# zoongahn/jodalroB-twoTower

Hardware: AMD Instinct MI355X
Metric: training pairs/sec at batch 8192 (embedding-lookup HBM GB/s in roofline) (higher is better)
Workload: dtype bf16 MFMA operands, f32 accumulate; f32 tables, master weights and activations (the tower input x, which the GEMMs round to bf16 anyway, is stored bf16)

## Files before the change

include/twotower.h:

```cpp
#ifndef TWOTOWER_H_
#define TWOTOWER_H_

#include <stddef.h>
#include <stdint.h>

#ifdef __cplusplus
extern "C" {
#endif

#define TT_ABI_VERSION 2

#define TT_OK 0
#define TT_ERR_INVALID_ARG (-1)
#define TT_ERR_HIP (-2)
#define TT_ERR_WORKSPACE (-3)
#define TT_ERR_UNSUPPORTED (-4)
#define TT_ERR_DEVICE (-5)

#define TT_F32 0
#define TT_BF16 1

#define TT_MAX_SIDES 4
#define TT_MAX_HIDDEN 8

// ... 15 lines not shown
#define TT_OPT_CHAINED 6
#define TT_OPT_LOOKUP_NT 7
#define TT_OPT_CHAIN_SPIN 8
#define TT_OPT_RETRIEVE_SPLITS 9
#define TT_OPT_FUSE_SCORE_TAIL 10
int tt_ctx_set_option(tt_ctx* ctx, int32_t option, int32_t value);
#define TT_DEVERR_CHAIN_TIMEOUT 1u
#define TT_DEVERR_ROW_RANGE 2u
int tt_ctx_check_device_errors(tt_ctx* ctx, tt_stream stream);
int tt_handover_retarget(tt_ctx* ctx, void* graph_exec, void* node);
int tt_handover_captured_node(tt_ctx* ctx, void** node);
int tt_flush_deferred(tt_ctx* ctx, tt_stream stream);
int tt_flush_deferred_slabs(tt_ctx* ctx, tt_stream stream);
int tt_deferred_pending(const tt_ctx* ctx);

typedef struct tt_embed_side {
  const int64_t* ids;
  const int64_t* key_row_offset;
  const int64_t* key_vocab;
  void* out;
  int64_t ld_out;
  int32_t K;
  int32_t out_dtype;
} tt_embed_side;

int tt_embed_lookup_set_profile(tt_ctx* ctx, uint64_t* ring_dev, int32_t n_slots);
int tt_embed_lookup_fwd(tt_ctx* ctx, const float* table, int64_t table_rows, int32_t E,
                        const tt_embed_side* sides, int32_t n_sides, int64_t B, int32_t* rows_out,
                        tt_stream stream);
int tt_embed_lookup_rows_fwd(tt_ctx* ctx, const float* table, int64_t table_rows, int32_t E,
                             const tt_embed_side* sides, int32_t n_sides, int64_t B, const int32_t* rows,
                             tt_stream stream);

size_t tt_dedup_workspace_bytes(int64_t M);
int tt_dedup_plan(tt_ctx* ctx, const int32_t* rows, int64_t M, int64_t table_rows,
                  int32_t* sorted_src, int32_t* unique_rows, int32_t* seg_offsets, int32_t* n_unique,
                  void* workspace, size_t workspace_bytes, tt_stream stream);

size_t tt_dedup_keyed_workspace_bytes(int64_t M, int32_t n_keys);
int tt_dedup_plan_keyed(tt_ctx* ctx, const int32_t* rows, const int32_t* side_K ,
                        int32_t n_sides, int64_t B, int32_t* sorted_src, int32_t* unique_rows,
                        int32_t* seg_offsets, int32_t* n_unique, void* workspace, size_t workspace_bytes,
                        tt_stream stream);

int tt_dedup_plan_keyed_km(tt_ctx* ctx, const int32_t* rows_km, const int32_t* side_K ,
                           int32_t n_sides, int64_t B, int32_t* sorted_src, int32_t* unique_rows,
                           int32_t* seg_offsets, int32_t* n_unique, void* workspace, size_t workspace_bytes,
                           tt_stream stream);

int tt_dedup_plan_keyed_long(tt_ctx* ctx, const int32_t* rows, int32_t rows_key_major, const int32_t* side_K ,
                             int32_t n_sides, int64_t B, int32_t E, int32_t* sorted_src, int32_t* unique_rows,
                             int32_t* seg_offsets, int32_t* n_unique, void* grad_workspace, size_t grad_workspace_bytes,
                             void* workspace, size_t workspace_bytes, tt_stream stream);

#define TT_GRAD_SPARSE 0
#define TT_GRAD_DENSE_SET 1
#define TT_GRAD_DENSE_ACC 2
#define TT_GRAD_SHORT_SEGMENTS 0x100
#define TT_GRAD_PLANNED 0x200
#define TT_GRAD_DEFER_FINISH 0x400

typedef struct tt_grad_src {
  const void* d_out;
  int64_t ld;
  int32_t K;
  int32_t dtype;
} tt_grad_src;

size_t tt_embed_grad_workspace_bytes(int64_t M, int32_t E);
int tt_embed_grad_bwd(tt_ctx* ctx, const tt_grad_src* srcs, int32_t n_srcs, int64_t B, int32_t E,
                      const int32_t* sorted_src, const int32_t* seg_offsets,
                      const int32_t* unique_rows, const int32_t* n_unique, int64_t M, int32_t mode,
                      float* out, int32_t* counters, void* workspace, size_t workspace_bytes, tt_stream stream);

void tt_adam_hparams(int64_t step, float lr, float beta1, float beta2, float eps, float weight_decay,
                     float out6[6]);
int tt_adam_dense_step(tt_ctx* ctx, float* p, const float* g, float* m, float* v, int64_t n,
                       int64_t step, float lr, float beta1, float beta2, float eps,
                       float weight_decay, const float* hparams_dev, tt_stream stream);
typedef struct tt_adam_tensor {
  float* p;
  const float* g;
  float* m;
  float* v;
  int64_t n;
} tt_adam_tensor;
int tt_adam_multi_step(tt_ctx* ctx, const tt_adam_tensor* tensors , int32_t n_tensors,
                       int64_t step, float lr, float beta1, float beta2, float eps,
                       float weight_decay, const float* hparams_dev, tt_stream stream);
int tt_sparse_adam_step(tt_ctx* ctx, float* table, float* m, float* v, int64_t table_rows, int32_t E,
                        const int32_t* unique_rows, const float* grad_rows, const int32_t* n_unique,
                        int64_t M, int64_t step, float lr, float beta1, float beta2, float eps,
                        float weight_decay, const float* hparams_dev, tt_stream stream);

int tt_adam_fused_step(tt_ctx* ctx, const tt_adam_tensor* tensors, int32_t n_tensors, float* table, float* m, float* v,
                       int64_t table_rows, int32_t E, const int32_t* unique_rows, const float* grad_rows, const int32_t* n_unique, int64_t M,
                       int64_t step, float lr, float beta1, float beta2, float eps, float weight_decay,
                       const float* hparams_dev, tt_stream stream);

int tt_adam_fused_step_finish(tt_ctx* ctx, const tt_adam_tensor* tensors, int32_t n_tensors, float* table, float* m, float* v,
                              int64_t table_rows, int32_t E, const int32_t* unique_rows, float* grad_rows, const int32_t* n_unique,
                              int64_t M, const int32_t* seg_offsets, void* grad_workspace, size_t grad_workspace_bytes,
                              int64_t step, float lr, float beta1, float beta2, float eps, float weight_decay,
                              const float* hparams_dev, tt_stream stream);

int tt_rowwise_adagrad_sparse_step(tt_ctx* ctx, float* table, float* sum, int64_t table_rows, int32_t E,
                                   const int32_t* unique_rows, const float* grad_rows, const int32_t* n_unique, int64_t M,
                                   float lr, float eps, float weight_decay, const float* hparams_dev, tt_stream stream);
int tt_rowwise_adagrad_dense_step(tt_ctx* ctx, float* table, float* sum, const float* grad, int64_t table_rows, int32_t E,
                                  float lr, float eps, float weight_decay, const float* hparams_dev, tt_stream stream);
int tt_adam_rowwise_adagrad_fused_step(tt_ctx* ctx, const tt_adam_tensor* tensors, int32_t n_tensors, int64_t step, float lr,
                                       float beta1, float beta2, float eps, float weight_decay, const float* hparams_dev,
                                       float* table, float* sum, int64_t table_rows, int32_t E, const int32_t* unique_rows,
                                       const float* grad_rows, const int32_t* n_unique, int64_t M, float table_lr,
                                       float table_eps, float table_weight_decay, const float* table_hparams_dev,
                                       tt_stream stream);
int tt_adam_rowwise_adagrad_fused_step_finish(tt_ctx* ctx, const tt_adam_tensor* tensors, int32_t n_tensors, int64_t step,
                                              float lr, float beta1, float beta2, float eps, float weight_decay,
                                              const float* hparams_dev, float* table, float* sum, int64_t table_rows, int32_t E,
                                              const int32_t* unique_rows, float* grad_rows, const int32_t* n_unique, int64_t M,
                                              const int32_t* seg_offsets, void* grad_workspace, size_t grad_workspace_bytes,
                                              float table_lr, float table_eps, float table_weight_decay,
                                              const float* table_hparams_dev, tt_stream stream);
int tt_embed_grad_finish(tt_ctx* ctx, int32_t E, const int32_t* seg_offsets, int64_t M, float* out, void* workspace,
                         size_t workspace_bytes, tt_stream stream);

typedef struct tt_tower_params {
  int32_t din, h0, kcat_e, n_hidden, d_out;
  int32_t hidden[TT_MAX_HIDDEN];
  const float* w_proj;
  const float* b_proj;
  const float* w[TT_MAX_HIDDEN];
  const float* b[TT_MAX_HIDDEN];
  const float* bn_w[TT_MAX_HIDDEN];
  const float* bn_b[TT_MAX_HIDDEN];
  float* bn_rm[TT_MAX_HIDDEN];
  float* bn_rv[TT_MAX_HIDDEN];
  int64_t* bn_nbt[TT_MAX_HIDDEN];
  const float* w_out;
  const float* b_out;
  int32_t compute_dtype;
  int32_t x_dtype;
  int32_t dx_dtype;
  int32_t flags;
  int32_t sync_phase;
  int32_t sync_ranks;
  int64_t rng_row_offset;
  const void* w_proj_bf16;
  const void* w_bf16[TT_MAX_HIDDEN];
} tt_tower_params;
#define TT_TOWER_UNFUSED_TAIL 1
#define TT_TOWER_UNFUSED_FRONT 2
#define TT_TOWER_UNFUSED_BACK 4

typedef struct tt_tower_acts {
  const float* dense;
  void* x;
  float* pre[TT_MAX_HIDDEN];
  float* act[TT_MAX_HIDDEN];
  float* mean[TT_MAX_HIDDEN];
  float* rstd[TT_MAX_HIDDEN];
  float* y;
  float* emb;
  void* emb_packed;
  float emb_pack_scale;
  float* bn_sync_local;
  const float* bn_sync_all;
  int64_t bn_sync_stride;
} tt_tower_acts;

typedef struct tt_tower_grads {
  float* w_proj;
  float* b_proj;
  float* w[TT_MAX_HIDDEN];
  float* b[TT_MAX_HIDDEN];
  float* bn_w[TT_MAX_HIDDEN];
  float* bn_b[TT_MAX_HIDDEN];
  float* w_out;
  float* b_out;
  void* d_x;
  float* scratch[TT_MAX_HIDDEN];
  float* d_y;
  float* s_sync_local;
  const float* s_sync_all;
  int64_t s_sync_stride;
} tt_tower_grads;

size_t tt_tower_workspace_bytes(const tt_tower_params* p, int64_t B);
int tt_tower_mlp_fwd(tt_ctx* ctx, const tt_tower_params* p, const tt_tower_acts* a, int64_t B,
                     int32_t train, float dropout_p, uint64_t seed, const uint64_t* seed_dev,
                     void* workspace, size_t workspace_bytes, tt_stream stream);
int tt_tower_mlp_bwd(tt_ctx* ctx, const tt_tower_params* p, const tt_tower_acts* a,
                     const float* d_emb, const tt_tower_grads* g, int64_t B, int32_t train,
                     float dropout_p, uint64_t seed, const uint64_t* seed_dev, void* workspace,
                     size_t workspace_bytes, tt_stream stream);

int tt_towers_mlp_fwd(tt_ctx* ctx, int32_t n, const tt_tower_params* const* p, const tt_tower_acts* const* a,
                      int64_t B, int32_t train, float dropout_p, uint64_t seed, const uint64_t* seed_dev,
                      void* const* workspaces, const size_t* workspace_bytes, tt_stream stream);
int tt_towers_mlp_bwd(tt_ctx* ctx, int32_t n, const tt_tower_params* const* p, const tt_tower_acts* const* a,
                      const float* const* d_emb, const tt_tower_grads* const* g, int64_t B, int32_t train,
                      float dropout_p, uint64_t seed, const uint64_t* seed_dev, void* const* workspaces,
                      const size_t* workspace_bytes, tt_stream stream);

int tt_score_dir_fwd(tt_ctx* ctx, const float* A, const float* Bm, int64_t Ra, int64_t Rb, int32_t D,
                     float inv_t, float shift, int64_t diag_offset, float* sumexp, float* diag,
                     int32_t* rank, float* sumscore ,
                     tt_stream stream);
int tt_score_loss_finish(tt_ctx* ctx, int64_t B, float shift, const float* rowsum,
                         const float* colsum, const float* diag, const int32_t* row_rank,
                         const int32_t* col_rank, const float* sumscore, float* out8,
                         float* loss_out , tt_stream stream);
int tt_score_dir_bwd(tt_ctx* ctx, const float* A, const float* Bm, int64_t Ra, int64_t Rb, int32_t D,
                     float inv_t, float shift, int64_t diag_offset, const float* sumexp_a,
                     const float* sumexp_b, const float* d_loss, float scale, float* dA,
                     tt_stream stream);
typedef struct tt_score_fwd_dir {
  const void* A_packed;
  const void* B_packed;
  int64_t Ra, Rb, diag_offset;
  float* sumexp;
  float* diag;
  int32_t* rank;
  float* sumscore;
  int32_t rank_mode;
  float ab_scale;
  float* inv_sumexp;
} tt_score_fwd_dir;
typedef struct tt_score_bwd_dir {
  const void* A_packed;
  const void* B_packed;
  int64_t Ra, Rb, diag_offset;
  const float* sumexp_a;
  const float* sumexp_b;
  float* dA;
  float ab_scale;
  float b_scale;
  const float* inv_a;
  const float* inv_b;
} tt_score_bwd_dir;
size_t tt_score_pack_bytes(int64_t R, int32_t D);
float tt_score_unit_scale(float inv_t);
int tt_score_pack_bf16(tt_ctx* ctx, const float* X, int64_t R, int32_t D, float scale, void* packed, tt_stream stream);
int tt_score_pack2_bf16(tt_ctx* ctx, const float* X0, int64_t R0, void* packed0, const float* X1, int64_t R1,
                        void* packed1, int32_t D, float scale0, float scale1, tt_stream stream);
int tt_score_fwd_bf16(tt_ctx* ctx, const tt_score_fwd_dir* dirs, int32_t n_dirs, int32_t D, float inv_t,
                      float shift, tt_stream stream);
int tt_score_bwd_bf16(tt_ctx* ctx, const tt_score_bwd_dir* dirs, int32_t n_dirs, int32_t D, float inv_t,
                      float shift, const float* d_loss, float scale, tt_stream stream);
size_t tt_score_fwd_sym_workspace_bytes(int64_t B, int32_t D);
int tt_score_fwd_sym_bf16(tt_ctx* ctx, const void* N_packed, const void* C_packed, int64_t B, int32_t D, float inv_t,
                          float shift, float ab_scale, int32_t want_rank, float* rowsum, float* colsum, float* inv_row,
                          float* inv_col, float* diag, int32_t* row_rank, float* out8, float* loss_out, void* workspace,
                          size_t workspace_bytes, tt_stream stream);
size_t tt_score_pack_fp8_bytes(int64_t R, int32_t D);
int tt_score_pack2_fp8(tt_ctx* ctx, const float* X0, int64_t R0, void* packed0, const float* X1, int64_t R1,
                       void* packed1, int32_t D, float scale0, float scale1, tt_stream stream);
int tt_score_fwd_sym_fp8(tt_ctx* ctx, const void* N_packed, const void* C_packed, int64_t B, int32_t D, float inv_t,
                         float shift, float ab_scale, int32_t want_rank, float* rowsum, float* colsum, float* inv_row,
                         float* inv_col, float* diag, int32_t* row_rank, float* out8, float* loss_out, void* workspace,
                         size_t workspace_bytes, tt_stream stream);
int tt_score_bwd_fp8(tt_ctx* ctx, const tt_score_bwd_dir* dirs, int32_t n_dirs, int32_t D, float inv_t,
                     float shift, const float* d_loss, float scale, tt_stream stream);
size_t tt_score_pack_x3_bytes(int64_t R, int32_t D);
int tt_score_pack2_bf16x3(tt_ctx* ctx, const float* X0, int64_t R0, void* packed0, const float* X1, int64_t R1,
                          void* packed1, int32_t D, float scale0, float scale1, tt_stream stream);
int tt_score_fwd_sym_bf16x3(tt_ctx* ctx, const void* N_packed, const void* C_packed, int64_t B, int32_t D, float inv_t,
                            float shift, float ab_scale, int32_t want_rank, float* rowsum, float* colsum, float* inv_row,
                            float* inv_col, float* diag, int32_t* row_rank, float* out8, float* loss_out, void* workspace,
                            size_t workspace_bytes, tt_stream stream);
int tt_score_fwd_bf16x3(tt_ctx* ctx, const tt_score_fwd_dir* dirs, int32_t n_dirs, int32_t D, float inv_t,
                        float shift, tt_stream stream);
int tt_score_bwd_bf16x3(tt_ctx* ctx, const tt_score_bwd_dir* dirs, int32_t n_dirs, int32_t D, float inv_t,
                        float shift, const float* d_loss, float scale, tt_stream stream);
typedef struct tt_score_bwd_lq {
  const float* w_a;
  const float* w_b;
} tt_score_bwd_lq;
int tt_score_fwd_sym_bf16_lq(tt_ctx* ctx, const void* N_packed, const void* C_packed, int64_t B, int32_t D, float inv_t,
                             float shift, float ab_scale, int32_t want_rank, const float* lq_n, const float* lq_c, float* rowsum,
                             float* colsum, float* inv_row, float* inv_col, float* w_n, float* w_c, float* diag,
                             int32_t* row_rank, float* out8, float* loss_out, void* workspace, size_t workspace_bytes,
                             tt_stream stream);
int tt_score_fwd_sym_bf16x3_lq(tt_ctx* ctx, const void* N_packed, const void* C_packed, int64_t B, int32_t D, float inv_t,
                               float shift, float ab_scale, int32_t want_rank, const float* lq_n, const float* lq_c,
                               float* rowsum, float* colsum, float* inv_row, float* inv_col, float* w_n, float* w_c,
                               float* diag, int32_t* row_rank, float* out8, float* loss_out, void* workspace,
                               size_t workspace_bytes, tt_stream stream);
int tt_score_bwd_bf16_lq(tt_ctx* ctx, const tt_score_bwd_dir* dirs, const tt_score_bwd_lq* lq, int32_t n_dirs, int32_t D,
                         float inv_t, float shift, const float* d_loss, float scale, tt_stream stream);
int tt_score_bwd_bf16x3_lq(tt_ctx* ctx, const tt_score_bwd_dir* dirs, const tt_score_bwd_lq* lq, int32_t n_dirs, int32_t D,
                           float inv_t, float shift, const float* d_loss, float scale, tt_stream stream);
int tt_score_dir_fwd_lq(tt_ctx* ctx, const float* A, const float* Bm, int64_t Ra, int64_t Rb, int32_t D, float inv_t,
                        float shift, int64_t diag_offset, const float* lq_b, float* sumexp, float* diag, int32_t* rank,
                        float* sumscore, tt_stream stream);
int tt_score_loss_finish_lq(tt_ctx* ctx, int64_t B, float shift, const float* lq_n, const float* lq_c, const float* rowsum,
                            const float* colsum, const float* diag, const int32_t* row_rank, const int32_t* col_rank,
                            const float* sumscore, float* out8, float* loss_out, tt_stream stream);
int tt_score_dir_bwd_lq(tt_ctx* ctx, const float* A, const float* Bm, int64_t Ra, int64_t Rb, int32_t D, float inv_t,
                        float shift, int64_t diag_offset, const float* lq_a, const float* lq_b, const float* sumexp_a,
                        const float* sumexp_b, const float* d_loss, float scale, float* dA, tt_stream stream);
int tt_score_fwd_sym_bf16_mask(tt_ctx* ctx, const void* N_packed, const void* C_packed, int64_t B, int32_t D, float inv_t,
                               float shift, float ab_scale, int32_t want_rank, const int32_t* ent_n, const int32_t* ent_c,
                               const float* lq_n, const float* lq_c, float* rowsum, float* colsum, float* inv_row,
                               float* inv_col, float* w_n, float* w_c, float* diag, int32_t* row_rank, float* out8,
                               float* loss_out, void* workspace, size_t workspace_bytes, tt_stream stream);
int tt_score_bwd_bf16_mask(tt_ctx* ctx, const tt_score_bwd_dir* dirs, const int32_t* ent_n, const int32_t* ent_c,
                           const tt_score_bwd_lq* lq, int32_t n_dirs, int32_t D, float inv_t, float shift,
                           const float* d_loss, float scale, tt_stream stream);
int tt_score_dir_fwd_mask(tt_ctx* ctx, const float* A, const float* Bm, int64_t Ra, int64_t Rb, int32_t D, float inv_t,
                          float shift, int64_t diag_offset, const int32_t* ent_n, const int32_t* ent_c, const float* lq_b,
                          float* sumexp, float* diag, int32_t* rank, float* sumscore, tt_stream stream);
int tt_score_dir_bwd_mask(tt_ctx* ctx, const float* A, const float* Bm, int64_t Ra, int64_t Rb, int32_t D, float inv_t,
                          float shift, int64_t diag_offset, const int32_t* ent_n, const int32_t* ent_c, const float* lq_a,
                          const float* lq_b, const float* sumexp_a, const float* sumexp_b, const float* d_loss, float scale,
                          float* dA, tt_stream stream);
int tt_score_prepare_pw(tt_ctx* ctx, const float* w, int64_t B, float* g_out, tt_stream stream);
int tt_score_fwd_sym_bf16_pw(tt_ctx* ctx, const void* N_packed, const void* C_packed, int64_t B, int32_t D, float inv_t,
                             float shift, float ab_scale, int32_t want_rank, const float* g, const int32_t* ent_n,
                             const int32_t* ent_c, const float* lq_n, const float* lq_c, float* rowsum, float* colsum,
                             float* inv_row, float* inv_col, float* w_n, float* w_c, float* diag, int32_t* row_rank,
                             float* out8, float* loss_out, void* workspace, size_t workspace_bytes, tt_stream stream);
int tt_score_bwd_bf16_pw(tt_ctx* ctx, const tt_score_bwd_dir* dirs, const float* g, const int32_t* ent_n,
                         const int32_t* ent_c, const tt_score_bwd_lq* lq, int32_t n_dirs, int32_t D, float inv_t, float shift,
                         const float* d_loss, float scale, tt_stream stream);
int tt_score_loss_finish_pw(tt_ctx* ctx, int64_t B, float shift, const float* g, const float* lq_n, const float* lq_c,
                            const float* rowsum, const float* colsum, const float* diag, const int32_t* row_rank,
                            const int32_t* col_rank, const float* sumscore, float* out8, float* loss_out, tt_stream stream);
int tt_score_dir_bwd_pw(tt_ctx* ctx, const float* A, const float* Bm, int64_t Ra, int64_t Rb, int32_t D, float inv_t,
                        float shift, int64_t diag_offset, const float* g, const int32_t* ent_n, const int32_t* ent_c,
                        const float* lq_a, const float* lq_b, const float* sumexp_a, const float* sumexp_b,
                        const float* d_loss, float scale, float* dA, tt_stream stream);
size_t tt_score_dense_workspace_bytes(int64_t B, int32_t D);
int tt_score_dense_fwd(tt_ctx* ctx, const float* N, const float* Cm, int64_t B, int32_t D, float inv_t, int32_t loss_type,
                       float label_smoothing, float* S, float* stats, int32_t* hit, float* out8, float* loss_out,
                       tt_stream stream);
int tt_score_dense_bwd(tt_ctx* ctx, const float* N, const float* Cm, int64_t B, int32_t D, float inv_t, int32_t loss_type,
                       float label_smoothing, float* S, const float* stats, const float* d_loss, float* dN, float* dC,
                       void* workspace, size_t workspace_bytes, tt_stream stream);
int tt_score_matrix(tt_ctx* ctx, const float* A, const float* Bm, int64_t Ra, int64_t Rb, int32_t D,
                    float inv_t, float* S, int64_t lds, tt_stream stream);
int tt_diag_rank_rows(tt_ctx* ctx, const float* S, int64_t R, int64_t Ccols, int64_t lds,
                      int64_t diag_offset, int32_t* rank, tt_stream stream);
int tt_topk_rows(tt_ctx* ctx, const float* S, int64_t R, int64_t Ccols, int64_t lds, int32_t k,
                 float* vals, int64_t* idx, tt_stream stream);

size_t tt_retrieve_workspace_bytes(int64_t nQ, int64_t nC, int32_t D, int32_t k);
int tt_retrieve_topk_bf16(tt_ctx* ctx, const void* Q_packed, int64_t nQ, const void* C_packed, int64_t nC, int32_t D, int32_t k,
                          const void* positives, int32_t positives_i64, float* vals, int64_t* idx, int32_t* rank, void* workspace,
                          size_t workspace_bytes, tt_stream stream);
int tt_retrieve_topk_f32(tt_ctx* ctx, const float* Q, int64_t nQ, const float* Cm, int64_t nC, int32_t D, float inv_t, int32_t k,
                         const void* positives, int32_t positives_i64, float* vals, int64_t* idx, int32_t* rank, void* workspace,
// ... 99 lines not shown
```

jodalrob-twotower_amd/_lib.py:

```python
from __future__ import annotations

import ctypes as C
from pathlib import Path
from typing import Optional

import torch

_PKG = Path(__file__).resolve().parent
LIB_PATH = _PKG / "libtwotower_hip.so"

TT_F32, TT_BF16 = 0, 1
TT_MAX_SIDES, TT_MAX_HIDDEN = 4, 8
TT_GRAD_SPARSE, TT_GRAD_DENSE_SET, TT_GRAD_DENSE_ACC = 0, 1, 2
TT_TOWER_UNFUSED_TAIL = 1
TT_TOWER_UNFUSED_FRONT = 2
TT_TOWER_UNFUSED_BACK = 4
TT_GRAD_SHORT_SEGMENTS = 0x100
TT_GRAD_PLANNED = 0x200
TT_GRAD_DEFER_FINISH = 0x400

vp = C.c_void_p
i32, i64, f32, u64, sz = C.c_int32, C.c_int64, C.c_float, C.c_uint64, C.c_size_t


class EmbedSide(C.Structure):
    _fields_ = [("ids", vp), ("key_row_offset", vp), ("key_vocab", vp), ("out", vp), ("ld_out", i64),
                ("K", i32), ("out_dtype", i32)]


class StoreSide(C.Structure):
    _fields_ = [("entity", vp), ("entity_stride", i64), ("dense_store", vp), ("cat_store", vp), ("dense_out", vp), ("ids_out", vp),
                ("dense_dim", i32), ("n_rows", i32)]


TT_MAX_CVT = 8


class CvtList(C.Structure):
    _fields_ = [("n", i32), ("reserved", i32), ("src", vp * TT_MAX_CVT), ("dst", vp * TT_MAX_CVT), ("count", i64 * TT_MAX_CVT)]


class IngestLookup(C.Structure):
    _fields_ = [("table", vp), ("table_rows", i64), ("E", i32), ("reserved", i32)]


class GradSrc(C.Structure):
    _fields_ = [("d_out", vp), ("ld", i64), ("K", i32), ("dtype", i32)]


class AdamTensor(C.Structure):
    _fields_ = [("p", vp), ("g", vp), ("m", vp), ("v", vp), ("n", i64)]


class ScoreFwdDir(C.Structure):
    _fields_ = [("A_packed", vp), ("B_packed", vp), ("Ra", i64), ("Rb", i64), ("diag_offset", i64),
                ("sumexp", vp), ("diag", vp), ("rank", vp), ("sumscore", vp), ("rank_mode", i32), ("ab_scale", f32), ("inv_sumexp", vp)]


class ScoreBwdDir(C.Structure):
    _fields_ = [("A_packed", vp), ("B_packed", vp), ("Ra", i64), ("Rb", i64), ("diag_offset", i64),
                ("sumexp_a", vp), ("sumexp_b", vp), ("dA", vp), ("ab_scale", f32), ("b_scale", f32), ("inv_a", vp), ("inv_b", vp)]


class ScoreBwdLq(C.Structure):
    _fields_ = [("w_a", vp), ("w_b", vp)]


_H = vp * TT_MAX_HIDDEN


class TowerParams(C.Structure):
    _fields_ = [("din", i32), ("h0", i32), ("kcat_e", i32), ("n_hidden", i32), ("d_out", i32),
                ("hidden", i32 * TT_MAX_HIDDEN),
                ("w_proj", vp), ("b_proj", vp), ("w", _H), ("b", _H), ("bn_w", _H), ("bn_b", _H),
                ("bn_rm", _H), ("bn_rv", _H), ("bn_nbt", _H), ("w_out", vp), ("b_out", vp), ("compute_dtype", i32),
                ("x_dtype", i32), ("dx_dtype", i32), ("flags", i32),
                ("sync_phase", i32), ("sync_ranks", i32), ("rng_row_offset", i64),
                ("w_proj_bf16", vp), ("w_bf16", _H)]


class TowerActs(C.Structure):
    _fields_ = [("dense", vp), ("x", vp), ("pre", _H), ("act", _H), ("mean", _H), ("rstd", _H), ("y", vp), ("emb", vp), ("emb_packed", vp), ("emb_pack_scale", f32),
                ("bn_sync_local", vp), ("bn_sync_all", vp), ("bn_sync_stride", i64)]


class TowerGrads(C.Structure):
    _fields_ = [("w_proj", vp), ("b_proj", vp), ("w", _H), ("b", _H), ("bn_w", _H), ("bn_b", _H),
                ("w_out", vp), ("b_out", vp), ("d_x", vp), ("scratch", _H), ("d_y", vp), ("s_sync_local", vp), ("s_sync_all", vp), ("s_sync_stride", i64)]


SIGNATURES = {
    "tt_abi_version": (C.c_int, []),
    "tt_ctx_create": (C.c_int, [C.c_int, C.POINTER(vp)]),
    "tt_ctx_destroy": (C.c_int, [vp]),
    "tt_last_error_string": (C.c_char_p, []),
    "tt_ctx_num_cus": (C.c_int, [vp]),
    "tt_embed_lookup_set_profile": (C.c_int, [vp, vp, i32]),
    "tt_embed_lookup_fwd": (C.c_int, [vp, vp, i64, i32, C.POINTER(EmbedSide), i32, i64, vp, vp]),
    "tt_embed_lookup_rows_fwd": (C.c_int, [vp, vp, i64, i32, C.POINTER(EmbedSide), i32, i64, vp, vp]),
    "tt_dedup_workspace_bytes": (sz, [i64]),
    "tt_dedup_plan": (C.c_int, [vp, vp, i64, i64, vp, vp, vp, vp, vp, sz, vp]),
    "tt_dedup_keyed_workspace_bytes": (sz, [i64, i32]),
    "tt_dedup_plan_keyed": (C.c_int, [vp, vp, C.POINTER(i32), i32, i64, vp, vp, vp, vp, vp, sz, vp]),
    "tt_dedup_plan_keyed_km": (C.c_int, [vp, vp, C.POINTER(i32), i32, i64, vp, vp, vp, vp, vp, sz, vp]),
    "tt_dedup_plan_keyed_long": (C.c_int, [vp, vp, i32, C.POINTER(i32), i32, i64, i32, vp, vp, vp, vp, vp, sz, vp, sz, vp]),
    "tt_embed_grad_workspace_bytes": (sz, [i64, i32]),
    "tt_embed_grad_bwd": (C.c_int, [vp, C.POINTER(GradSrc), i32, i64, i32, vp, vp, vp, vp, i64, i32, vp, vp, vp, sz, vp]),
    "tt_adam_hparams": (None, [i64, f32, f32, f32, f32, f32, C.POINTER(f32 * 6)]),
    "tt_adam_dense_step": (C.c_int, [vp, vp, vp, vp, vp, i64, i64, f32, f32, f32, f32, f32, vp, vp]),
    "tt_adam_multi_step": (C.c_int, [vp, C.POINTER(AdamTensor), i32, i64, f32, f32, f32, f32, f32, vp, vp]),
    "tt_sparse_adam_step": (C.c_int, [vp, vp, vp, vp, i64, i32, vp, vp, vp, i64, i64, f32, f32, f32, f32, f32, vp, vp]),
    "tt_adam_fused_step": (C.c_int, [vp, C.POINTER(AdamTensor), i32, vp, vp, vp, i64, i32, vp, vp, vp, i64, i64, f32, f32, f32, f32,
                                     f32, vp, vp]),
    "tt_adam_fused_step_finish": (C.c_int, [vp, C.POINTER(AdamTensor), i32, vp, vp, vp, i64, i32, vp, vp, vp, i64, vp, vp, sz, i64, f32,
                                            f32, f32, f32, f32, vp, vp]),
    "tt_rowwise_adagrad_sparse_step": (C.c_int, [vp, vp, vp, i64, i32, vp, vp, vp, i64, f32, f32, f32, vp, vp]),
    "tt_rowwise_adagrad_dense_step": (C.c_int, [vp, vp, vp, vp, i64, i32, f32, f32, f32, vp, vp]),
    "tt_adam_rowwise_adagrad_fused_step": (C.c_int, [vp, C.POINTER(AdamTensor), i32, i64, f32, f32, f32, f32, f32, vp, vp, vp, i64, i32,
                                                     vp, vp, vp, i64, f32, f32, f32, vp, vp]),
    "tt_adam_rowwise_adagrad_fused_step_finish": (C.c_int, [vp, C.POINTER(AdamTensor), i32, i64, f32, f32, f32, f32, f32, vp, vp, vp,
                                                            i64, i32, vp, vp, vp, i64, vp, vp, sz, f32, f32, f32, vp, vp]),
    "tt_embed_grad_finish": (C.c_int, [vp, i32, vp, i64, vp, vp, sz, vp]),
    "tt_ctx_set_option": (C.c_int, [vp, i32, i32]),
    "tt_flush_deferred": (C.c_int, [vp, vp]),
    "tt_ctx_check_device_errors": (C.c_int, [vp, vp]),
    "tt_handover_retarget": (C.c_int, [vp, vp, vp]),
    "tt_handover_captured_node": (C.c_int, [vp, C.POINTER(vp)]),
    "tt_deferred_pending": (C.c_int, [vp]),
    "tt_launch_count": (C.c_uint64, []),
    "tt_flush_deferred_slabs": (C.c_int, [vp, vp]),
    "tt_tower_workspace_bytes": (sz, [C.POINTER(TowerParams), i64]),
    "tt_tower_mlp_fwd": (C.c_int, [vp, C.POINTER(TowerParams), C.POINTER(TowerActs), i64, i32, f32, u64, vp, vp, sz, vp]),
    "tt_tower_mlp_bwd": (C.c_int, [vp, C.POINTER(TowerParams), C.POINTER(TowerActs), vp, C.POINTER(TowerGrads), i64, i32,
                                   f32, u64, vp, vp, sz, vp]),
    "tt_towers_mlp_fwd": (C.c_int, [vp, i32, C.POINTER(C.POINTER(TowerParams)), C.POINTER(C.POINTER(TowerActs)), i64, i32, f32, u64,
                                    vp, C.POINTER(vp), C.POINTER(sz), vp]),
    "tt_towers_mlp_bwd": (C.c_int, [vp, i32, C.POINTER(C.POINTER(TowerParams)), C.POINTER(C.POINTER(TowerActs)), C.POINTER(vp),
                                    C.POINTER(C.POINTER(TowerGrads)), i64, i32, f32, u64, vp, C.POINTER(vp), C.POINTER(sz), vp]),
    "tt_score_dir_fwd": (C.c_int, [vp, vp, vp, i64, i64, i32, f32, f32, i64, vp, vp, vp, vp, vp]),
    "tt_score_loss_finish": (C.c_int, [vp, i64, f32, vp, vp, vp, vp, vp, vp, vp, vp, vp]),
    "tt_score_dir_bwd": (C.c_int, [vp, vp, vp, i64, i64, i32, f32, f32, i64, vp, vp, vp, f32, vp, vp]),
    "tt_score_pack_bytes": (sz, [i64, i32]),
    "tt_score_unit_scale": (f32, [f32]),
    "tt_score_pack_bf16": (C.c_int, [vp, vp, i64, i32, f32, vp, vp]),
    "tt_score_pack2_bf16": (C.c_int, [vp, vp, i64, vp, vp, i64, vp, i32, f32, f32, vp]),
    "tt_score_fwd_bf16": (C.c_int, [vp, C.POINTER(ScoreFwdDir), i32, i32, f32, f32, vp]),
    "tt_score_bwd_bf16": (C.c_int, [vp, C.POINTER(ScoreBwdDir), i32, i32, f32, f32, vp, f32, vp]),
    "tt_score_pack_fp8_bytes": (sz, [i64, i32]),
    "tt_score_pack2_fp8": (C.c_int, [vp, vp, i64, vp, vp, i64, vp, i32, f32, f32, vp]),
    "tt_score_fwd_sym_fp8": (C.c_int, [vp, vp, vp, i64, i32, f32, f32, f32, i32, vp, vp, vp, vp, vp, vp, vp, vp, vp, sz, vp]),
    "tt_score_bwd_fp8": (C.c_int, [vp, C.POINTER(ScoreBwdDir), i32, i32, f32, f32, vp, f32, vp]),
    "tt_score_fwd_sym_workspace_bytes": (sz, [i64, i32]),
    "tt_score_fwd_sym_bf16": (C.c_int, [vp, vp, vp, i64, i32, f32, f32, f32, i32, vp, vp, vp, vp, vp, vp, vp, vp, vp, sz, vp]),
    "tt_score_pack_x3_bytes": (sz, [i64, i32]),
    "tt_score_pack2_bf16x3": (C.c_int, [vp, vp, i64, vp, vp, i64, vp, i32, f32, f32, vp]),
    "tt_score_fwd_sym_bf16x3": (C.c_int, [vp, vp, vp, i64, i32, f32, f32, f32, i32, vp, vp, vp, vp, vp, vp, vp, vp, vp, sz, vp]),
    "tt_score_fwd_bf16x3": (C.c_int, [vp, C.POINTER(ScoreFwdDir), i32, i32, f32, f32, vp]),
    "tt_score_bwd_bf16x3": (C.c_int, [vp, C.POINTER(ScoreBwdDir), i32, i32, f32, f32, vp, f32, vp]),
    "tt_score_fwd_sym_bf16_lq": (C.c_int, [vp, vp, vp, i64, i32, f32, f32, f32, i32, vp, vp, vp, vp, vp, vp, vp, vp, vp, vp, vp, vp, vp,
                                           sz, vp]),
    "tt_score_fwd_sym_bf16x3_lq": (C.c_int, [vp, vp, vp, i64, i32, f32, f32, f32, i32, vp, vp, vp, vp, vp, vp, vp, vp, vp, vp, vp, vp, vp,
                                             sz, vp]),
    "tt_score_bwd_bf16_lq": (C.c_int, [vp, C.POINTER(ScoreBwdDir), C.POINTER(ScoreBwdLq), i32, i32, f32, f32, vp, f32, vp]),
    "tt_score_bwd_bf16x3_lq": (C.c_int, [vp, C.POINTER(ScoreBwdDir), C.POINTER(ScoreBwdLq), i32, i32, f32, f32, vp, f32, vp]),
    "tt_score_dir_fwd_lq": (C.c_int, [vp, vp, vp, i64, i64, i32, f32, f32, i64, vp, vp, vp, vp, vp, vp]),
    "tt_score_loss_finish_lq": (C.c_int, [vp, i64, f32, vp, vp, vp, vp, vp, vp, vp, vp, vp, vp, vp]),
    "tt_score_dir_bwd_lq": (C.c_int, [vp, vp, vp, i64, i64, i32, f32, f32, i64, vp, vp, vp, vp, vp, f32, vp, vp]),
    "tt_score_fwd_sym_bf16_mask": (C.c_int, [vp, vp, vp, i64, i32, f32, f32, f32, i32, vp, vp, vp, vp, vp, vp, vp, vp, vp, vp, vp, vp, vp,
                                             vp, vp, sz, vp]),
    "tt_score_bwd_bf16_mask": (C.c_int, [vp, C.POINTER(ScoreBwdDir), vp, vp, C.POINTER(ScoreBwdLq), i32, i32, f32, f32, vp, f32, vp]),
    "tt_score_dir_fwd_mask": (C.c_int, [vp, vp, vp, i64, i64, i32, f32, f32, i64, vp, vp, vp, vp, vp, vp, vp, vp]),
    "tt_score_dir_bwd_mask": (C.c_int, [vp, vp, vp, i64, i64, i32, f32, f32, i64, vp, vp, vp, vp, vp, vp, vp, f32, vp, vp]),
    "tt_score_prepare_pw": (C.c_int, [vp, vp, i64, vp, vp]),
    "tt_score_fwd_sym_bf16_pw": (C.c_int, [vp, vp, vp, i64, i32, f32, f32, f32, i32, vp, vp, vp, vp, vp, vp, vp, vp, vp, vp, vp, vp, vp, vp,
                                           vp, vp, sz, vp]),
    "tt_score_bwd_bf16_pw": (C.c_int, [vp, C.POINTER(ScoreBwdDir), vp, vp, vp, C.POINTER(ScoreBwdLq), i32, i32, f32, f32, vp, f32, vp]),
    "tt_score_loss_finish_pw": (C.c_int, [vp, i64, f32, vp, vp, vp, vp, vp, vp, vp, vp, vp, vp, vp, vp]),
    "tt_score_dir_bwd_pw": (C.c_int, [vp, vp, vp, i64, i64, i32, f32, f32, i64, vp, vp, vp, vp, vp, vp, vp, vp, f32, vp, vp]),
    "tt_score_matrix": (C.c_int, [vp, vp, vp, i64, i64, i32, f32, vp, i64, vp]),
    "tt_score_dense_workspace_bytes": (sz, [i64, i32]),
    "tt_score_dense_fwd": (C.c_int, [vp, vp, vp, i64, i32, f32, i32, f32, vp, vp, vp, vp, vp, vp]),
    "tt_score_dense_bwd": (C.c_int, [vp, vp, vp, i64, i32, f32, i32, f32, vp, vp, vp, vp, vp, vp, sz, vp]),
    "tt_diag_rank_rows": (C.c_int, [vp, vp, i64, i64, i64, i64, vp, vp]),
    "tt_topk_rows": (C.c_int, [vp, vp, i64, i64, i64, i32, vp, vp, vp]),
    "tt_retrieve_workspace_bytes": (sz, [i64, i64, i32, i32]),
    "tt_retrieve_topk_bf16": (C.c_int, [vp, vp, i64, vp, i64, i32, i32, vp, i32, vp, vp, vp, vp, sz, vp]),
    "tt_retrieve_topk_f32": (C.c_int, [vp, vp, i64, vp, i64, i32, f32, i32, vp, i32, vp, vp, vp, vp, sz, vp]),
    "tt_excl_retrieve_topk_bf16": (C.c_int, [vp, vp, i64, vp, i64, i32, i32, vp, i32, vp, vp, vp, vp, vp, vp, sz, vp]),
    "tt_excl_retrieve_topk_f32": (C.c_int, [vp, vp, i64, vp, i64, i32, f32, i32, vp, i32, vp, vp, vp, vp, vp, vp, sz, vp]),
    "tt_filt_retrieve_topk_bf16": (C.c_int, [vp, vp, i64, vp, i64, i32, i32, vp, i32, vp, vp, vp, vp, vp, vp, i32, vp, vp, vp, sz, vp]),
    "tt_filt_retrieve_topk_f32": (C.c_int, [vp, vp, i64, vp, i64, i32, f32, i32, vp, i32, vp, vp, vp, vp, vp, vp, i32, vp, vp, vp, sz,
                                            vp]),
    "tt_linear_fwd": (C.c_int, [vp, vp, i64, vp, vp, vp, i64, i64, i32, i32, i32, vp]),
    "tt_route_workspace_bytes": (sz, [i64, i32]),
    "tt_route_bucket": (C.c_int, [vp, vp, vp, i64, i32, i32, C.POINTER(i32), i32, vp, vp, vp, vp, vp, vp, sz, vp]),
    "tt_route_expand": (C.c_int, [vp, vp, vp, vp, vp, i64, vp, vp]),
    "tt_route_bucket_expand": (C.c_int, [vp, vp, vp, i64, i32, i32, C.POINTER(i32), i32, vp, vp, vp, vp, vp, vp, sz, vp, vp, vp, vp]),
    "tt_dedup_plan_runs": (C.c_int, [vp, vp, i32, i64, i64, vp, vp, vp, vp, vp, sz, vp]),
    "tt_gather_rows": (C.c_int, [vp, vp, i64, i32, vp, i64, vp, i32, vp]),
    "tt_copy_multi": (C.c_int, [vp, i32, C.POINTER(vp), C.POINTER(vp), C.POINTER(i64), vp]),
    "tt_batch_ingest": (C.c_int, [vp, i32, C.POINTER(vp), C.POINTER(vp), C.POINTER(i64), C.POINTER(EmbedSide), i32, i64, vp, vp, i64, C.POINTER(CvtList), vp]),
    "tt_batch_gather": (C.c_int, [vp, vp, i64, vp, i32, vp, i32, vp, vp, vp]),
    "tt_batch_ingest_store": (C.c_int, [vp, i32, C.POINTER(vp), C.POINTER(vp), C.POINTER(i64), C.POINTER(EmbedSide), C.POINTER(StoreSide), i32,
                                        i64, vp, vp, vp, i64, C.POINTER(CvtList), vp]),
    "tt_batch_ingest_lookup": (C.c_int, [vp, i32, C.POINTER(vp), C.POINTER(vp), C.POINTER(i64), C.POINTER(EmbedSide), i32, i64, vp,
                                         C.POINTER(IngestLookup), C.POINTER(CvtList), vp]),
    "tt_batch_ingest_store_lookup": (C.c_int, [vp, i32, C.POINTER(vp), C.POINTER(vp), C.POINTER(i64), C.POINTER(EmbedSide), C.POINTER(StoreSide),
                                               i32, i64, vp, vp, C.POINTER(IngestLookup), C.POINTER(CvtList), vp]),
}

_lib: Optional[C.CDLL] = None
_ctxs: dict = {}
_defer_on: set = set()
_riders_on: dict = {}
_workspaces: dict = {}


class TwoTowerHipError(RuntimeError):
    pass


def load() -> C.CDLL:
    global _lib
    if _lib is None:
        if not LIB_PATH.exists():
            raise TwoTowerHipError(
                f"{LIB_PATH} is missing: build it with `python -c 'import __graft_entry__ as g; g.build()'` "
                "(hipcc --offload-arch=gfx950).  There is no CPU fallback for the two-tower hot path.")
        lib = C.CDLL(str(LIB_PATH))
        for name, (res, args) in SIGNATURES.items():
            fn = getattr(lib, name)
            fn.restype, fn.argtypes = res, args
        _lib = lib
    return _lib


def check(rc: int, what: str = ""):
    if rc != 0:
        msg = load().tt_last_error_string().decode("utf-8", "replace")
        raise TwoTowerHipError(f"{what or 'twotower call'} failed (status {rc}): {msg}")


def ctx(device: torch.device) -> vp:
    device = torch.device(device)
    if device.type != "cuda":
        raise TwoTowerHipError(f"the two-tower hot path runs on MI355X only; got tensors on '{device}' "
                               "(no CPU fallback exists)")
    idx = device.index if device.index is not None else torch.cuda.current_device()
    if idx not in _ctxs:
        h = vp()
        check(load().tt_ctx_create(idx, C.byref(h)), "tt_ctx_create")
        _ctxs[idx] = h
    return _ctxs[idx]


def stream(device: torch.device) -> vp:
    return vp(torch.cuda.current_stream(device).cuda_stream)


def ptr(t: Optional[torch.Tensor]) -> vp:
    return vp(0 if t is None else t.data_ptr())


TT_OPT_DEFER_SLAB_REDUCE = 1
TT_OPT_KEYED_PARTS = 2
TT_OPT_SCORE_BWD_ROWS_MIN = 3
TT_OPT_DEFER_RIDERS = 4
TT_OPT_FP8_GRAD = 5
TT_OPT_CHAINED = 6
TT_OPT_LOOKUP_NT = 7
TT_OPT_CHAIN_SPIN = 8
TT_OPT_RETRIEVE_SPLITS = 9
TT_OPT_FUSE_SCORE_TAIL = 10


def set_option(device: torch.device, option: int, value: int):
    check(load().tt_ctx_set_option(ctx(device), int(option), int(value)), "tt_ctx_set_option")


def set_defer_slab_reduce(device: torch.device, on: bool):
    check(load().tt_ctx_set_option(ctx(device), TT_OPT_DEFER_SLAB_REDUCE, 1 if on else 0), "tt_ctx_set_option")
    idx = torch.device(device).index
    (_defer_on.add if on else _defer_on.discard)(idx if idx is not None else torch.cuda.current_device())
    if not on:
        flush_deferred(device)


def set_defer_riders(device: torch.device, on, loss_only: bool = False):
    mask = (2 if loss_only else 3) if on else 0
# ... 78 lines not shown
```

jodalrob-twotower_amd/config.py:

```python
from __future__ import annotations

import os
from dataclasses import dataclass


@dataclass
class Settings:
    score_dtype: str = "fp32"
    mlp_dtype: str = "fp32"
    embedding_grad: str = "dense"
    sync_debug: bool = False
    tower_io_dtype: str = "x"
    tower_unfused_tail: bool = False
    tower_unfused_front: bool = False
    tower_unfused_back: bool = False
    tower_pack: bool = True
    graph_ingest: bool = True
    graph_weight_shadows: bool = True
    graph_ingest_rows: bool = True
    graph_ingest_lookup: bool = False
    grad_planned: bool = True

    @classmethod
    def from_env(cls) -> "Settings":
        e = os.environ
        return cls(score_dtype=e.get("TT_SCORE_DTYPE", "fp32"), mlp_dtype=e.get("TT_MLP_DTYPE", "fp32"),
                   embedding_grad=e.get("TT_EMBEDDING_GRAD", "dense"), sync_debug=e.get("TT_SYNC_DEBUG", "0") not in ("", "0"))


settings = Settings.from_env()
```

jodalrob-twotower_amd/csrc/tt_tower.hip:

```cpp
#include "tt_deferred.h"
#include "tt_tail_bwd.h"

namespace {

using namespace tttail;

constexpr int kThreads = 256;

struct BnStatArgs {
  const float* pre; int B, H, rows_per_chunk, nchunks; float* partial; float* mean; float* rstd; float* rm; float* rv; int64_t* nbt;
  int64_t pstride = 0;
};

__global__ __launch_bounds__(kThreads) void bn_stats_partial_kernel(Batch<BnStatArgs> batch) {
  const BnStatArgs& a = batch.a[blockIdx.z];
  const int H = a.H;
  if ((int)blockIdx.x * 64 >= H || (int)blockIdx.y >= a.nchunks) return;
  __shared__ Wf sh[4][64];
  const int c = blockIdx.x * 64 + (threadIdx.x & 63), rl = threadIdx.x >> 6;
  const int r0 = blockIdx.y * a.rows_per_chunk, r1 = min(a.B, r0 + a.rows_per_chunk);
  Wf w{0.f, 0.f, 0.f};
  if (c < H && r0 + rl < r1) {
    const float x0 = fmaxf(a.pre[(int64_t)(r0 + rl) * H + c], 0.f);
    float s = 0.f, q = 0.f, cnt = 0.f;
// ... 217 lines not shown
  for (int r = 0; r < RW; ++r)
#pragma unroll
    for (int j = 0; j < NC; ++j) v[r][j] = row0 + r < a.B ? a.y[(int64_t)(row0 + r) * D + lane + 64 * j] : 0.f;
#pragma unroll
  for (int r = 0; r < RW; ++r) {
    float ss = mul_rn(v[r][0], v[r][0]);
#pragma unroll
    for (int j = 1; j < NC; ++j) ss = __builtin_fmaf(v[r][j], v[r][j], ss);
    const float den = fmaxf(sqrtf(wave_sum(ss)), kNormEps);
    if (row0 + r < a.B) {
#pragma unroll
      for (int j = 0; j < NC; ++j) a.out[(int64_t)(row0 + r) * D + lane + 64 * j] = v[r][j] / den;
    }
  }
}

template <int NC, int RW>
__global__ __launch_bounds__(kThreads) void l2norm_bwd_fast_kernel(Batch<NormArgs> batch) {
  const NormArgs& a = batch.a[blockIdx.y];
  const int lane = threadIdx.x & 63, D = 64 * NC;
  const int row0 = (blockIdx.x * 4 + (threadIdx.x >> 6)) * RW;
  if (row0 >= a.B) return;
  float y[RW][NC], e[RW][NC], d[RW][NC];
#pragma unroll
  for (int r = 0; r < RW; ++r)
#pragma unroll
    for (int j = 0; j < NC; ++j) {
      const bool ok = row0 + r < a.B;
      const int64_t i = (int64_t)(row0 + r) * D + lane + 64 * j;
      y[r][j] = ok ? a.y[i] : 0.f;
      e[r][j] = ok ? a.emb_in[i] : 0.f;
      d[r][j] = ok ? a.d_emb[i] : 0.f;
    }
#pragma unroll
  for (int r = 0; r < RW; ++r) {
    float ss = mul_rn(y[r][0], y[r][0]), dot = mul_rn(e[r][0], d[r][0]);
#pragma unroll
    for (int j = 1; j < NC; ++j) {
      ss = __builtin_fmaf(y[r][j], y[r][j], ss);
      dot = __builtin_fmaf(e[r][j], d[r][j], dot);
    }
    const float nrm = sqrtf(wave_sum(ss));
    dot = wave_sum(dot);
    const float den = fmaxf(nrm, kNormEps);
    if (row0 + r < a.B) {
#pragma unroll
      for (int j = 0; j < NC; ++j)
        a.out[(int64_t)(row0 + r) * D + lane + 64 * j] = nrm > kNormEps ? (d[r][j] - e[r][j] * dot) / den : d[r][j] / den;
    }
  }
}

template <bool BWD>
static bool launch_l2norm_fast(hipStream_t st, const Batch<NormArgs>& na, int n, int64_t B) {
  const int D = na.a[0].D;
  for (int t = 1; t < n; ++t)
    if (na.a[t].D != D || na.a[t].B != na.a[0].B) return false;
  if (D % 64 != 0 || D < 64 || D > 256) return false;
  constexpr int RW = BWD ? 2 : 4;
  const dim3 grid((unsigned)tt_cdiv(B, 4 * RW), (unsigned)n);
  auto launch = [&](auto kernel) { kernel<<<grid, kThreads, 0, st>>>(na); };
#define TT_L2(NC)                                        \
  do {                                                   \
    if (BWD) launch(l2norm_bwd_fast_kernel<NC, RW>);     \
    else launch(l2norm_fwd_fast_kernel<NC, RW>);         \
  } while (0)
  switch (D / 64) {
    case 1: TT_L2(1); break;
    case 2: TT_L2(2); break;
    case 3: TT_L2(3); break;
    default: TT_L2(4); break;
  }
#undef TT_L2
  return true;
}

constexpr int kTailThreads = 1024;

struct HeadArgs { const float* slabs; int64_t slab_stride; int splits; const float* bias; float* pre; BnStatArgs s; };

__global__ __launch_bounds__(kTailThreads) void tail_head_kernel(Batch<HeadArgs> batch) {
  const HeadArgs& h = batch.a[blockIdx.y];
  const BnStatArgs& a = h.s;
  const int H = a.H;
  if ((int)blockIdx.x >= a.nchunks) return;
  __shared__ float X[64 * kTailLdF];
  __shared__ Wf sh[4][64];
  const int t = threadIdx.x, c = t & 63, rq = t >> 6;
  const int r0 = blockIdx.x * a.rows_per_chunk, r1 = min(a.B, r0 + a.rows_per_chunk);
  const float bias = (h.bias && c < H) ? h.bias[c] : 0.f;
  float x0 = 0.f, s = 0.f, q = 0.f, cnt = 0.f;
  for (int b0 = r0; b0 < r1; b0 += 64) {
    float v[4] = {0.f, 0.f, 0.f, 0.f};
    if (c < H) {
#pragma unroll 4
      for (int z = 0; z < h.splits; ++z) {
#pragma unroll
        for (int j = 0; j < 4; ++j) {
          const int r = b0 + rq + 16 * j;
          if (r < r1) v[j] += h.slabs[(int64_t)z * h.slab_stride + (int64_t)r * H + c];
        }
      }
#pragma unroll
      for (int j = 0; j < 4; ++j) {
        const int row = rq + 16 * j, r = b0 + row;
        if (r < r1) {
          const float o = v[j] + bias;
          h.pre[(int64_t)r * H + c] = o;
          X[row * kTailLdF + c] = fmaxf(o, 0.f);
        }
      }
    }
    __syncthreads();
    if (t < 256 && c < H) {
      const int nrow = min(64, r1 - b0);
      for (int row = rq; row < nrow; row += 4) {
        const float xv = X[row * kTailLdF + c];
        if (cnt == 0.f) x0 = xv;
        const float d = xv - x0;
        s += d;
        q += d * d;
        cnt += 1.f;
      }
    }
    __syncthreads();
  }
  if (t < 256) {
    Wf w{0.f, 0.f, 0.f};
    if (c < H && cnt > 0.f) {
      w.n = cnt;
      w.mean = x0 + s / cnt;
      w.m2 = fmaxf(q - s * (s / cnt), 0.f);
    }
    sh[rq][c] = w;
  }
  __syncthreads();
  if (t < 64 && c < H) {
    Wf o = sh[0][c];
    o = wf_combine(o, sh[1][c]);
    o = wf_combine(o, sh[2][c]);
    o = wf_combine(o, sh[3][c]);
    float* p = a.partial + (int64_t)blockIdx.x * 3 * H;
    p[c] = o.n; p[H + c] = o.mean; p[2 * H + c] = o.m2;
  }
}

struct FrontArgs {
  const float* dense; int64_t ld_dense; int din;
  const float* w_proj; const float* b_proj; int h0;
  uint16_t* x; int64_t ldx; int kx;
  const float* w; const float* bias; float* pre;
  BnStatArgs s;
  const uint16_t* w_proj16; const uint16_t* w16;
};
constexpr int kFS = 136;
constexpr int kFrontThreads = 512;
constexpr int kFrontA = 64 * kFS * 2, kFrontB = 128 * kFS * 2;
constexpr int kFrontLds = 2 * kFrontA + 2 * kFrontB + kFrontA + 4 * 64 * 12;

using tl_bf16x4 = __attribute__((ext_vector_type(4))) __bf16;
__device__ __forceinline__ void front_put4(__bf16* dst, const float4& v, bool live) {
  tl_bf16x4 o;
  o[0] = (__bf16)(live ? v.x : 0.f); o[1] = (__bf16)(live ? v.y : 0.f);
  o[2] = (__bf16)(live ? v.z : 0.f); o[3] = (__bf16)(live ? v.w : 0.f);
  *reinterpret_cast<tl_bf16x4*>(dst) = o;
}

template <typename T>
__device__ __forceinline__ T front_ld(const void* base, uint32_t off) {
  return *reinterpret_cast<const T*>(reinterpret_cast<const char*>(base) + off);
}

template <bool W16>
__global__ __launch_bounds__(kFrontThreads) void tower_front_kernel(Batch<FrontArgs> batch) {
  const FrontArgs& f = batch.a[blockIdx.y];
  const BnStatArgs& a = f.s;
  const int H = a.H, B = a.B, h0 = f.h0, din = f.din, kx = f.kx;
  if ((int)blockIdx.x >= a.nchunks) return;
  extern __shared__ __attribute__((aligned(16))) char front_smem[];
  __bf16* bufA = reinterpret_cast<__bf16*>(front_smem);
  __bf16* bufB = reinterpret_cast<__bf16*>(front_smem + 2 * kFrontA);
  __bf16* Pt = reinterpret_cast<__bf16*>(front_smem + 2 * kFrontA + 2 * kFrontB);
  Wf (*sh)[64] = reinterpret_cast<Wf (*)[64]>(front_smem + 3 * kFrontA + 2 * kFrontB);
  float* part = reinterpret_cast<float*>(bufB);
  const int t = threadIdx.x, lane = t & 63, wave = t >> 6, li = lane & 31, lh = lane >> 5;
  const int c = t & 63, rq = t >> 6;
  const int r0 = blockIdx.x * a.rows_per_chunk, r1 = min(B, r0 + a.rows_per_chunk);
  const float bias = (f.bias && c < H) ? f.bias[c] : 0.f;
  const int frow = t >> 5, fk = 4 * (t & 31), xrow = t >> 4, xk = 8 * (t & 15);
  const int fkp = din >= 128 ? fk : (fk & 63), fkb = kx >= 128 ? fk : (fk & 63), xkb = kx >= 128 ? xk : (xk & 63);
  const int xkp = din >= 128 ? xk : (xk & 63);
  const int ns2 = 3 * ((kx + 383) / 384);
  const int pn = (wave >> 1) * 32 + li;
  const float bp = pn < h0 ? f.b_proj[pn] : 0.f;
  float x0 = 0.f, s = 0.f, q = 0.f, cnt = 0.f;
  for (int b0 = r0; b0 < r1; b0 += 64) {
    constexpr int NPB = W16 ? 4 : 8, NQB = W16 ? 2 : 4;
    float4 pa[2][4], pb[2][NPB];
    uint32_t oa[4], ob[NPB];
#pragma unroll
    for (int ps = 0; ps < 4; ++ps) oa[ps] = (uint32_t)(min(b0 + frow + 16 * ps, B - 1) * (int)f.ld_dense + fkp) * 4u;
#pragma unroll
    for (int ps = 0; ps < NPB; ++ps)
      ob[ps] = W16 ? (uint32_t)(min(xrow + 32 * ps, h0 - 1) * din + xkp) * 2u : (uint32_t)(min(frow + 16 * ps, h0 - 1) * din + fkp) * 4u;
#pragma unroll
    for (int st = 0; st < 2; ++st) {
      const uint32_t ko = 128 * st + fk < din ? 512u * st : 0u;
      const uint32_t ko16 = 128 * st + xk < din ? 256u * st : 0u;
#pragma unroll
      for (int ps = 0; ps < 4; ++ps) pa[st][ps] = front_ld<float4>(f.dense, oa[ps] + ko);
#pragma unroll
      for (int ps = 0; ps < NPB; ++ps) pb[st][ps] = W16 ? front_ld<float4>(f.w_proj16, ob[ps] + ko16) : front_ld<float4>(f.w_proj, ob[ps] + ko);
    }
    uint4 qa[3][2];
    float4 qb[3][NQB];
    uint32_t ox[2], ow[NQB];
#pragma unroll
    for (int ps = 0; ps < 2; ++ps) ox[ps] = (uint32_t)(min(b0 + xrow + 32 * ps, B - 1) * (int)f.ldx + xkb) * 2u;
#pragma unroll
    for (int ps = 0; ps < NQB; ++ps)
      ow[ps] = W16 ? (uint32_t)(min(xrow + 32 * ps, H - 1) * kx + xkb) * 2u : (uint32_t)(min(frow + 16 * ps, H - 1) * kx + fkb) * 4u;
#pragma unroll
    for (int u = 0; u < 2; ++u) {
      const int ka = 128 * u + xk, kb = 128 * u + fk;
#pragma unroll
      for (int ps = 0; ps < 2; ++ps) qa[u][ps] = front_ld<uint4>(f.x, ox[ps] + (ka < kx ? 256u * u : 0u));
#pragma unroll
      for (int ps = 0; ps < NQB; ++ps)
        qb[u][ps] = W16 ? front_ld<float4>(f.w16, ow[ps] + (ka < kx ? 256u * u : 0u)) : front_ld<float4>(f.w, ow[ps] + (kb < kx ? 512u * u : 0u));
    }
    __builtin_amdgcn_sched_barrier(0);
    {
      const int rt = wave & 1, ct = wave >> 1;
      tl_f32x16 acc;
#pragma unroll
      for (int i = 0; i < 16; ++i) acc[i] = 0.f;
#pragma unroll
      for (int st = 0; st < 2; ++st) {
        const bool live = 128 * st + fk < din, live16 = 128 * st + xk < din;
#pragma unroll
        for (int ps = 0; ps < 4; ++ps) front_put4(bufA + st * 64 * kFS + (frow + 16 * ps) * kFS + fk, pa[st][ps], live);
#pragma unroll
        for (int ps = 0; ps < NPB; ++ps) {
          if (W16) *reinterpret_cast<float4*>(bufB + st * 128 * kFS + (xrow + 32 * ps) * kFS + xk) = live16 ? pb[st][ps] : float4{0.f, 0.f, 0.f, 0.f};
          else front_put4(bufB + st * 128 * kFS + (frow + 16 * ps) * kFS + fk, pb[st][ps], live);
        }
      }
      {
        const int ka = 256 + xk, kb = 256 + fk;
#pragma unroll
        for (int ps = 0; ps < 2; ++ps) qa[2][ps] = front_ld<uint4>(f.x, ox[ps] + (ka < kx ? 512u : 0u));
#pragma unroll
        for (int ps = 0; ps < NQB; ++ps)
          qb[2][ps] = W16 ? front_ld<float4>(f.w16, ow[ps] + (ka < kx ? 512u : 0u)) : front_ld<float4>(f.w, ow[ps] + (kb < kx ? 1024u : 0u));
      }
      __syncthreads();
#pragma unroll
      for (int st = 0; st < 2; ++st) {
        const __bf16* A = bufA + st * 64 * kFS;
        const __bf16* Bm = bufB + st * 128 * kFS;
        if (128 * st < din) {
#pragma unroll
          for (int s2 = 0; s2 < 8; ++s2) {
            const int k = 16 * s2 + 8 * lh;
            const tl_bf16x8 av = *reinterpret_cast<const tl_bf16x8*>(A + (rt * 32 + li) * kFS + k);
            const tl_bf16x8 bv = *reinterpret_cast<const tl_bf16x8*>(Bm + (ct * 32 + li) * kFS + k);
            acc = __builtin_amdgcn_mfma_f32_32x32x16_bf16(av, bv, acc, 0, 0, 0);
          }
        }
      }
#pragma unroll
      for (int r = 0; r < 16; ++r) {
        const int m = rt * 32 + (r & 3) + 8 * (r >> 2) + 4 * lh;
        if (pn < h0) Pt[m * kFS + pn] = (__bf16)(acc[r] + bp);
      }
      __syncthreads();
#pragma unroll
      for (int ps = 0; ps < 2; ++ps)
        if (xk < h0 && b0 + xrow + 32 * ps < r1)
          *reinterpret_cast<uint4*>(f.x + (int64_t)(b0 + xrow + 32 * ps) * f.ldx + xk) =
              *reinterpret_cast<const uint4*>(Pt + (xrow + 32 * ps) * kFS + xk);
    }
    {
      const int tile = wave & 3, kq = wave >> 2, rt = tile & 1, nh = tile >> 1;
      tl_f32x16 acc;
#pragma unroll
      for (int i = 0; i < 16; ++i) acc[i] = 0.f;
      for (int s0 = 0; s0 < ns2; s0 += 3) {
#pragma unroll
        for (int u = 0; u < 3; ++u) {
          const int st = s0 + u;
          __bf16* A = bufA + (st & 1) * 64 * kFS;
          __bf16* Bm = bufB + (st & 1) * 128 * kFS;
#pragma unroll
          for (int ps = 0; ps < 2; ++ps)
            *reinterpret_cast<uint4*>(A + (xrow + 32 * ps) * kFS + xk) = (128 * st + xk < kx) ? qa[u][ps] : uint4{0u, 0u, 0u, 0u};
#pragma unroll
          for (int ps = 0; ps < NQB; ++ps) {
            if (W16) *reinterpret_cast<float4*>(Bm + (xrow + 32 * ps) * kFS + xk) = (128 * st + xk < kx) ? qb[u][ps] : float4{0.f, 0.f, 0.f, 0.f};
            else front_put4(Bm + (frow + 16 * ps) * kFS + fk, qb[u][ps], 128 * st + fk < kx);
          }
          __syncthreads();
          {
            const int ka = 128 * (st + 3) + xk, kb = 128 * (st + 3) + fk;
#pragma unroll
            for (int ps = 0; ps < 2; ++ps) qa[u][ps] = front_ld<uint4>(f.x, ox[ps] + (ka < kx ? 256u * (uint32_t)(st + 3) : 0u));
#pragma unroll
            for (int ps = 0; ps < NQB; ++ps)
              qb[u][ps] = W16 ? front_ld<float4>(f.w16, ow[ps] + (ka < kx ? 256u * (uint32_t)(st + 3) : 0u))
                              : front_ld<float4>(f.w, ow[ps] + (kb < kx ? 512u * (uint32_t)(st + 3) : 0u));
          }
#pragma unroll
          for (int s2 = 0; s2 < 4; ++s2) {
            const int kl = 16 * (4 * kq + s2), kglob = 128 * st + kl;
            const __bf16* asrc = kglob < h0 ? Pt + (rt * 32 + li) * kFS + kglob + 8 * lh : A + (rt * 32 + li) * kFS + kl + 8 * lh;
            const tl_bf16x8 av = *reinterpret_cast<const tl_bf16x8*>(asrc);
            const tl_bf16x8 bv = *reinterpret_cast<const tl_bf16x8*>(Bm + (nh * 32 + li) * kFS + kl + 8 * lh);
            acc = __builtin_amdgcn_mfma_f32_32x32x16_bf16(av, bv, acc, 0, 0, 0);
          }
        }
      }
      __syncthreads();
      const int n = nh * 32 + li;
#pragma unroll
      for (int r = 0; r < 16; ++r) part[(kq * 64 + rt * 32 + (r & 3) + 8 * (r >> 2) + 4 * lh) * 64 + n] = acc[r];
    }
    __syncthreads();
    if (c < H) {
      float v[8];
#pragma unroll
      for (int j = 0; j < 8; ++j) {
        const int row = rq + 8 * j;
        v[j] = (part[row * 64 + c] + part[(64 + row) * 64 + c]) + bias;
      }
#pragma unroll
      for (int j = 0; j < 8; ++j) {
        const int row = rq + 8 * j, r = b0 + row;
        if (r < r1) f.pre[(int64_t)r * H + c] = v[j];
        part[row * 64 + c] = fmaxf(v[j], 0.f);
      }
    }
    __syncthreads();
    if (t < 256 && c < H) {
      const int nrow = min(64, r1 - b0);
      for (int row = rq; row < nrow; row += 4) {
        const float xv = part[row * 64 + c];
        if (cnt == 0.f) x0 = xv;
        const float d = xv - x0;
        s += d;
        q += d * d;
        cnt += 1.f;
      }
    }
    __syncthreads();
  }
  if (t < 256) {
    Wf w{0.f, 0.f, 0.f};
    if (c < H && cnt > 0.f) {
      w.n = cnt;
      w.mean = x0 + s / cnt;
      w.m2 = fmaxf(q - s * (s / cnt), 0.f);
    }
    sh[rq][c] = w;
  }
  __syncthreads();
  if (t < 64 && c < H) {
    Wf o = sh[0][c];
    o = wf_combine(o, sh[1][c]);
    o = wf_combine(o, sh[2][c]);
    o = wf_combine(o, sh[3][c]);
    float* p = a.partial + (int64_t)blockIdx.x * 3 * H;
    p[c] = o.n; p[H + c] = o.mean; p[2 * H + c] = o.m2;
  }
}

struct TailFwdArgs {
  BnStatArgs s;
  const float* g; const float* b; uint64_t salt; float* act;
  const float* w_out; const float* b_out; int D; float* y; float* emb;
  __bf16* pk_rows; __bf16* pk_frag; int Dp; float pk_scale;
  const float* fin = nullptr;
};

static_assert(kTailThreads == kRiderThreads, "the riders run in the tail kernels' workgroups");
#ifdef TT_TAIL_STAMPS
__device__ unsigned long long g_tail_stamps[2][512 * 8];
#define TT_TAIL_STAMP(k, i) do { if (threadIdx.x == 0) g_tail_stamps[k][((blockIdx.y * gridDim.x + blockIdx.x) & 511) * 8 + (i)] = __builtin_amdgcn_s_memrealtime(); } while (0)
#else
#define TT_TAIL_STAMP(k, i) do { } while (0)
#endif

template <bool FIN>
__global__ __launch_bounds__(kTailThreads) __attribute__((amdgpu_waves_per_eu(8, 8)))
void tail_fwd_kernel(Batch<TailFwdArgs> batch, bool drop, float p, uint64_t seed0,
                     const uint64_t* __restrict__ seed_dev, CompactRider cr, int cr_wg) {
  if (cr_wg > 0 && blockIdx.y == 0) {
    if ((int)blockIdx.x < cr_wg) compact_body(cr, blockIdx.x);
    return;
  }
  const TailFwdArgs& f = batch.a[blockIdx.y - (cr_wg > 0 ? 1 : 0)];
  const BnStatArgs& a = f.s;
  const int H = a.H, D = f.D, B = a.B;
  const int m0 = blockIdx.x * 64;
  if (m0 >= B) return;
  TT_TAIL_STAMP(0, 0);
  __shared__ Wf sh[FIN ? 1 : 16][64];
  __shared__ float s_mean[64], s_rstd[64];
  __shared__ __attribute__((aligned(16))) __bf16 As[64 * kTailLd];
  __shared__ __attribute__((aligned(16))) __bf16 Bs[64 * kTailLd];
  __shared__ float Y[64 * kTailLdF];
  const int t = threadIdx.x, c = t & 63, rq = t >> 6;
  float pre[4];
#pragma unroll
  for (int j = 0; j < 4; ++j) {
    const int r = m0 + rq + 16 * j;
    const float v = a.pre[(int64_t)min(r, B - 1) * H + min(c, H - 1)];
    pre[j] = (c < H && r < B) ? v : 0.f;
  }
  float fm = 0.f, fr = 0.f;
  if (FIN) {
    const float v0 = f.fin[min(c, H - 1)], v1 = f.fin[H + min(c, H - 1)];
    fm = c < H ? v0 : 0.f;
    fr = c < H ? v1 : 0.f;
  } else {
    sh[rq][c] = bn_finish_subchain(a.partial, a.pstride ? a.pstride : 3 * H, a.nchunks, H, c, rq);
  }
#pragma unroll
  for (int j = 0; j < 4; ++j) {
    const int n = rq + 16 * j;
    const float w = f.w_out[(int64_t)min(n, D - 1) * H + min(c, H - 1)];
    Bs[n * kTailLd + c] = (__bf16)((n < D && c < H) ? w : 0.f);
  }
  if (!FIN) {
    __syncthreads();
    TT_TAIL_STAMP(0, 1);
    if (t < 64 && c < H) {
      bn_finish_column(sh, c, blockIdx.x == 0, a.mean, a.rstd, a.rm, a.rv, a.nbt, fm, fr);
      s_mean[c] = fm;
      s_rstd[c] = fr;
    }
    __syncthreads();
  } else {
    TT_TAIL_STAMP(0, 1);
  }
  TT_TAIL_STAMP(0, 2);
  {
    const uint64_t seed = drop ? seed_of(seed0, seed_dev) : 0;
    const float mean = FIN ? fm : (c < H ? s_mean[c] : 0.f), rstd = FIN ? fr : (c < H ? s_rstd[c] : 0.f);
    const float g = c < H ? f.g[c] : 0.f, bb = c < H ? f.b[c] : 0.f;
#pragma unroll
    for (int j = 0; j < 4; ++j) {
      const int row = rq + 16 * j, r = m0 + row;
      float v = 0.f;
      if (c < H && r < B) {
        const int64_t i = (int64_t)r * H + c;
        const float x = fmaxf(pre[j], 0.f);
        const float yv = (x - mean) * rstd * g + bb;
        v = yv * dropout_scale(drop, p, seed, f.salt + (uint64_t)i);
        f.act[i] = v;
// ... 492 lines not shown
  const BnBwdArgs& b = ta.bn;
  const int H = a.H, B = a.B;
  const int t = threadIdx.x, c = t & 255, rq = t >> 8;
  const int m0 = blockIdx.x * 64;
  if (m0 >= B) return;
  __shared__ float sh[2][4][kWideH];
  float pr[16], da[16];
#pragma unroll
  for (int j = 0; j < 16; ++j) {
    const int64_t i = (int64_t)min(m0 + rq + 4 * j, B - 1) * H + min(c, H - 1);
    pr[j] = b.pre[i];
    da[j] = b.d[i];
  }
  float s0 = 0.f, s1 = 0.f;
  {
    const int64_t ps = a.pstride ? a.pstride : 2 * H;
    const int cc = min(c, H - 1);
#pragma unroll
    for (int half = 0; half < 2; ++half) {
      float v0[kMaxChunks / 8], v1[kMaxChunks / 8];
#pragma unroll
      for (int i = 0; i < kMaxChunks / 8; ++i) {
        const int k = rq + 4 * (i + half * (kMaxChunks / 8));
        const float* q = a.partial + (int64_t)min(k, a.nchunks - 1) * ps;
        const float x0 = q[cc], x1 = q[H + cc];
        v0[i] = k < a.nchunks ? x0 : 0.f;
        v1[i] = k < a.nchunks ? x1 : 0.f;
      }
#pragma unroll
      for (int i = 0; i < kMaxChunks / 8; ++i) { s0 += v0[i]; s1 += v1[i]; }
    }
  }
  sh[0][rq][c] = s0;
  sh[1][rq][c] = s1;
  __syncthreads();
  if (c < H) {
    const float S1 = (sh[0][0][c] + sh[0][1][c]) + (sh[0][2][c] + sh[0][3][c]);
    const float S2 = (sh[1][0][c] + sh[1][1][c]) + (sh[1][2][c] + sh[1][3][c]);
    if (blockIdx.x == 0 && rq == 0) { a.out0[c] = S1 * ta.out_scale; a.out1[c] = S2 * ta.out_scale; }
    const float mean = b.mean[c], rstd = b.rstd[c], g = b.g[c];
#pragma unroll
    for (int j = 0; j < 16; ++j) {
      const int r = m0 + rq + 4 * j;
      if (r < B) {
        const float xh = (fmaxf(pr[j], 0.f) - mean) * rstd;
        const float dv = g * rstd * (da[j] - S1 * b.invB - xh * (S2 * b.invB));
        b.d[(int64_t)r * H + c] = pr[j] > 0.f ? dv : 0.f;
      }
    }
  }
}

struct LocalArgs { const float* partial; int nchunks, H; float* out; };

__global__ __launch_bounds__(kThreads) void tail_local_stats_kernel(Batch<LocalArgs> batch) {
  const LocalArgs& a = batch.a[blockIdx.y];
  const int H = a.H;
  if ((int)blockIdx.x * 64 >= H) return;
  __shared__ Wf sh[4][64];
  const int cl = threadIdx.x & 63, c = blockIdx.x * 64 + cl, jl = threadIdx.x >> 6;
  Wf o{0.f, 0.f, 0.f};
  if (c < H) {
    Wf v[kMaxChunks / 4];
#pragma unroll
    for (int i = 0; i < kMaxChunks / 4; ++i) {
      const int k = jl + 4 * i;
      const float* q = a.partial + (int64_t)k * 3 * H;
      v[i] = k < a.nchunks ? Wf{q[c], q[H + c], q[2 * H + c]} : Wf{0.f, 0.f, 0.f};
    }
    o = wf_lane_merge(v);
  }
  sh[jl][cl] = o;
  __syncthreads();
  if (jl == 0 && c < H) {
    o = wf_combine(wf_combine(sh[0][cl], sh[1][cl]), wf_combine(sh[2][cl], sh[3][cl]));
    a.out[c] = o.n; a.out[H + c] = o.mean; a.out[2 * H + c] = o.m2;
  }
}

__global__ __launch_bounds__(kThreads) void tail_local_colsum_kernel(Batch<LocalArgs> batch) {
  const LocalArgs& a = batch.a[blockIdx.y];
  const int H = a.H;
  if ((int)blockIdx.x * 64 >= H) return;
  __shared__ float sh[2][4][64];
  const int cl = threadIdx.x & 63, c = blockIdx.x * 64 + cl, jl = threadIdx.x >> 6;
  float s0 = 0.f, s1 = 0.f;
  if (c < H) {
    float v0[kMaxChunks / 4], v1[kMaxChunks / 4];
#pragma unroll
    for (int i = 0; i < kMaxChunks / 4; ++i) {
      const int k = jl + 4 * i;
      const float* q = a.partial + (int64_t)k * 2 * H;
      v0[i] = k < a.nchunks ? q[c] : 0.f;
      v1[i] = k < a.nchunks ? q[H + c] : 0.f;
    }
#pragma unroll
    for (int i = 0; i < kMaxChunks / 4; ++i) { s0 += v0[i]; s1 += v1[i]; }
  }
  sh[0][jl][cl] = s0;
  sh[1][jl][cl] = s1;
  __syncthreads();
  if (jl == 0 && c < H) {
    a.out[c] = (sh[0][0][cl] + sh[0][1][cl]) + (sh[0][2][cl] + sh[0][3][cl]);
    a.out[H + c] = (sh[1][0][cl] + sh[1][1][cl]) + (sh[1][2][cl] + sh[1][3][cl]);
  }
}

inline int ew_grid(const tt_ctx* ctx, int64_t n, int towers) {
  const int64_t cap = (int64_t)ctx->num_cus * 8 / (towers > 0 ? towers : 1);
  int64_t b = tt_cdiv(n, kThreads);
  return (int)(b < 1 ? 1 : (b < cap ? b : cap));
}

inline int chunks_for(int64_t B, int H) {
  int64_t n = 512 / tt_cdiv(H, 64);
  if (n > kMaxChunks) n = kMaxChunks;
  const int64_t mx = tt_cdiv(B, 64);
  if (n > mx) n = mx;
  return (int)(n < 1 ? 1 : n);
}

struct WsLayout {
  char* gemm;
  size_t gemm_bytes;
  char* tn[TT_MAX_HIDDEN + 2];
  size_t tn_bytes[TT_MAX_HIDDEN + 2];
  float* col;
  size_t col_bytes;
  size_t total;
};

inline int in_width(const tt_tower_params* p, int i) { return i == 0 ? p->h0 + p->kcat_e : p->hidden[i - 1]; }
inline int last_width(const tt_tower_params* p) { return p->n_hidden == 0 ? p->h0 + p->kcat_e : p->hidden[p->n_hidden - 1]; }

inline bool tail_shape_ok(const tt_tower_params* p) {
  return p->n_hidden >= 1 && p->hidden[p->n_hidden - 1] <= 64 && p->d_out <= 64;
}
inline bool tail_fusable(int n, const tt_tower_params* const* P, int train) {
  if (!train || P[0]->compute_dtype != TT_BF16) return false;
  for (int t = 0; t < n; ++t)
    if (!tail_shape_ok(P[t]) || (P[t]->flags & TT_TOWER_UNFUSED_TAIL)) return false;
  return true;
}
inline bool front_fusable(int n, const tt_tower_params* const* P, const tt_tower_acts* const* A) {
  for (int t = 0; t < n; ++t) {
    const tt_tower_params* p = P[t];
    const int kx = p->h0 + p->kcat_e;
    if (p->n_hidden != 1 || p->x_dtype != TT_BF16 || (p->flags & TT_TOWER_UNFUSED_FRONT)) return false;
    if (p->h0 % 32 != 0 || p->h0 > 128 || p->din % 64 != 0 || p->din > 256 || kx % 64 != 0) return false;
    if (!tt_aligned(A[t]->dense, 16) || !tt_aligned(A[t]->x, 16) || !tt_aligned(p->w_proj, 16) || !tt_aligned(p->w[0], 16)) return false;
  }
  return true;
}
inline bool wide_tail_ok(int n, const tt_tower_params* const* P, int train) {
  if (!train || P[0]->compute_dtype != TT_BF16) return false;
  for (int t = 0; t < n; ++t) {
    const tt_tower_params* p = P[t];
    if (p->n_hidden < 1 || p->hidden[p->n_hidden - 1] > kWideH || p->d_out > kWideD || (p->flags & TT_TOWER_UNFUSED_TAIL)) return false;
  }
  return true;
}
inline size_t tail_slab_bytes(const tt_tower_params* p) {
  return sizeof(float) * (size_t)kMaxChunks * ((size_t)p->d_out * p->hidden[p->n_hidden - 1] + (size_t)p->d_out) + 256;
}

inline WsLayout ws_layout(const tt_tower_params* p, int64_t B, char* base) {
  size_t g = tt_gemm_tn_workspace_bytes(p->h0, p->din, B);
  int hmax = p->d_out > p->h0 ? p->d_out : p->h0;
  for (int i = 0; i < p->n_hidden; ++i) {
    const size_t b = tt_gemm_tn_workspace_bytes(p->hidden[i], in_width(p, i), B);
    g = b > g ? b : g;
    hmax = p->hidden[i] > hmax ? p->hidden[i] : hmax;
  }
  const size_t b = tt_gemm_tn_workspace_bytes(p->d_out, last_width(p), B);
  g = b > g ? b : g;
  {
    int nmax = p->h0 > p->d_out ? p->h0 : p->d_out;
    for (int i = 0; i < p->n_hidden; ++i) nmax = p->hidden[i] > nmax ? p->hidden[i] : nmax;
    const size_t f = tt_gemm_nt_workspace_bytes(B, nmax, 0);
    g = f > g ? f : g;
  }
  WsLayout w;
  w.gemm_bytes = (g + 255) & ~size_t(255);
  w.col_bytes = sizeof(float) * 3 * (size_t)hmax * (size_t)kMaxChunks + 256;
  w.gemm = base;
  w.col = reinterpret_cast<float*>(base ? base + w.gemm_bytes : nullptr);
  size_t o = w.gemm_bytes + ((w.col_bytes + 255) & ~size_t(255));
  for (int l = 0; l < p->n_hidden + 2; ++l) {
    size_t nb = l == 0 ? tt_gemm_tn_workspace_bytes(p->h0, p->din, B)
              : l == p->n_hidden + 1 ? tt_gemm_tn_workspace_bytes(p->d_out, last_width(p), B)
                                     : tt_gemm_tn_workspace_bytes(p->hidden[l - 1], in_width(p, l - 1), B);
    if (l == p->n_hidden + 1 && tail_shape_ok(p) && tail_slab_bytes(p) > nb) nb = tail_slab_bytes(p);
    if (l == 0 && p->n_hidden >= 1) {
      const size_t gb = tt_gemm_back_g_workspace_bytes(p->hidden[0], p->h0, p->din, B);
      nb = gb > nb ? gb : nb;
    }
    w.tn[l] = base ? base + o : nullptr;
    w.tn_bytes[l] = (nb + 255) & ~size_t(255);
    o += w.tn_bytes[l];
  }
  w.total = o;
  return w;
}

int check_params(const tt_tower_params* p, const char* who) {
  TT_CHECK_ARG(p, "%s: params NULL", who);
  TT_CHECK_ARG(p->n_hidden >= 0 && p->n_hidden <= TT_MAX_HIDDEN, "%s: n_hidden=%d not in [0,%d]", who, p->n_hidden, TT_MAX_HIDDEN);
  TT_CHECK_ARG(p->din >= 1 && p->h0 >= 1 && p->kcat_e >= 0 && p->d_out >= 1, "%s: bad dims", who);
  TT_CHECK_ARG(p->w_proj && p->b_proj && p->w_out && p->b_out, "%s: NULL projection/output weights", who);
  for (int i = 0; i < p->n_hidden; ++i) {
    TT_CHECK_ARG(p->hidden[i] >= 1, "%s: hidden[%d] < 1", who, i);
    TT_CHECK_ARG(p->w[i] && p->b[i] && p->bn_w[i] && p->bn_b[i] && p->bn_rm[i] && p->bn_rv[i], "%s: NULL block %d params", who, i);
  }
  return TT_OK;
}

int check_batch(int32_t n, const tt_tower_params* const* P, int64_t B, float dropout_p, void* const* ws, const size_t* wsb,
                const char* who) {
  TT_CHECK_ARG(n >= 1 && n <= TT_MAX_SIDES && P && ws && wsb, "%s: need 1..%d towers", who, TT_MAX_SIDES);
  TT_CHECK_ARG(B >= 0 && B < ((int64_t)1 << 24), "%s: B=%lld out of range", who, (long long)B);
  TT_CHECK_ARG(dropout_p >= 0.f && dropout_p < 1.f, "%s: dropout_p=%f not in [0,1)", who, dropout_p);
  for (int t = 0; t < n; ++t) {
    if (int rc = check_params(P[t], who)) return rc;
    TT_CHECK_ARG(P[t]->n_hidden == P[0]->n_hidden, "%s: towers fused into one launch must have the same number of hidden blocks", who);
    TT_CHECK_ARG(P[t]->compute_dtype == P[0]->compute_dtype, "%s: towers fused into one launch must share compute_dtype", who);
    TT_CHECK_ARG((P[t]->x_dtype == TT_F32 && P[t]->dx_dtype == TT_F32) || P[t]->compute_dtype == TT_BF16,
                 "%s: bf16 x / d_x need compute_dtype TT_BF16", who);
    TT_CHECK_ARG((P[t]->x_dtype == TT_F32 || P[t]->x_dtype == TT_BF16) && (P[t]->dx_dtype == TT_F32 || P[t]->dx_dtype == TT_BF16),
                 "%s: bad x_dtype / dx_dtype", who);
    TT_CHECK_ARG(P[t]->sync_phase == P[0]->sync_phase && P[t]->sync_phase >= 0 && P[t]->sync_phase <= 2, "%s: bad / mixed sync_phase", who);
    TT_CHECK_ARG(P[t]->sync_phase == 0 || (P[t]->sync_ranks >= 1 && P[t]->sync_ranks <= kMaxChunks), "%s: sync_ranks=%d not in [1, %d]", who,
                 P[t]->sync_ranks, kMaxChunks);
    if (B > 0 && (!ws[t] || wsb[t] < tt_tower_workspace_bytes(P[t], B))) {
      tt_set_error("%s: workspace of tower %d: %zu < required %zu", who, t, wsb[t], tt_tower_workspace_bytes(P[t], B));
      return TT_ERR_WORKSPACE;
    }
  }
  return TT_OK;
}

struct Pass {
  tt_ctx* ctx; hipStream_t st; int n;
  const tt_tower_params* const* P; const tt_tower_acts* const* A; const tt_tower_grads* const* G; const float* const* d_emb;
  int64_t B; WsLayout ws[TT_MAX_SIDES];
  bool train, drop; float dropout_p; uint64_t seed; const uint64_t* seed_dev;
  int phase, nh; bool bf16;
};
inline Pass make_pass(tt_ctx* ctx, tt_stream stream, int n, const tt_tower_params* const* P, const tt_tower_acts* const* A,
                      const tt_tower_grads* const* G, const float* const* d_emb, int64_t B, int32_t train, float dropout_p, uint64_t seed,
                      const uint64_t* seed_dev, void* const* workspaces) {
  Pass p{ctx, reinterpret_cast<hipStream_t>(stream), n, P, A, G, d_emb, B, {}, train != 0, train && dropout_p > 0.f, dropout_p, seed, seed_dev,
         P[0]->sync_phase, P[0]->n_hidden, P[0]->compute_dtype == TT_BF16};
  for (int t = 0; t < n; ++t) p.ws[t] = ws_layout(P[t], B, reinterpret_cast<char*>(workspaces[t]));
  return p;
}
int check_sync_phase(const Pass& p, const char* who) {
  if (p.phase == 0) return TT_OK;
  if (p.nh != 1 || !p.train) {
    tt_set_error("%s: sync_phase %d needs a training pass over towers with exactly one hidden block (the pass is cut at its BatchNorm)", who, p.phase);
    return TT_ERR_UNSUPPORTED;
  }
  for (int t = 0; t < p.n; ++t) {
    const float* buf = p.G ? (!p.G[t] ? nullptr : p.phase == 1 ? p.G[t]->s_sync_local : p.G[t]->s_sync_all)
                           : (p.phase == 1 ? p.A[t]->bn_sync_local : p.A[t]->bn_sync_all);
    TT_CHECK_ARG(buf != nullptr, "%s: NULL SyncBN buffer", who);
  }
  return TT_OK;
}
inline uint64_t block_salt(const tt_tower_params* p, int t, int i) {
  return (((uint64_t)(i + 1) << 40) ^ ((uint64_t)t << 52)) + (uint64_t)p->rng_row_offset * (uint64_t)p->hidden[i];
}
inline const float* layer_in(const Pass& p, int i, int t) { return i == 0 ? reinterpret_cast<const float*>(p.A[t]->x) : p.A[t]->act[i - 1]; }
inline float* d_in(const Pass& p, int i, int t) { return i == 0 ? reinterpret_cast<float*>(p.G[t]->d_x) : p.G[t]->scratch[i - 1]; }
inline int block_chunks(const Pass& p, int i, int t) { return chunks_for(p.B, p.P[t]->hidden[i]); }
struct BlockDims { int hmax = 1, cmax = 1; int64_t tmax = 1; };
inline BlockDims block_dims(const Pass& p, int i) {
  BlockDims d;
  for (int t = 0; t < p.n; ++t) {
    const int H = p.P[t]->hidden[i], nchunks = block_chunks(p, i, t);
    d.hmax = H > d.hmax ? H : d.hmax;
    d.cmax = nchunks > d.cmax ? nchunks : d.cmax;
    d.tmax = p.B * H > d.tmax ? p.B * H : d.tmax;
  }
  return d;
}
inline BnStatArgs bn_stat_args(const Pass& p, int i, int t) {
  const tt_tower_params* P = p.P[t]; const tt_tower_acts* A = p.A[t];
  const int nchunks = block_chunks(p, i, t);
  return BnStatArgs{A->pre[i], (int)p.B, P->hidden[i], (int)tt_cdiv(p.B, nchunks), nchunks, p.ws[t].col, A->mean[i], A->rstd[i],
                    P->bn_rm[i], P->bn_rv[i], P->bn_nbt[i]};
}
inline BnApplyArgs bn_apply_args(const Pass& p, int i, int t) {
  const tt_tower_params* P = p.P[t]; const tt_tower_acts* A = p.A[t];
  return BnApplyArgs{A->pre[i], p.B * P->hidden[i], P->hidden[i], A->mean[i], A->rstd[i], P->bn_w[i], P->bn_b[i], block_salt(P, t, i), A->act[i]};
}
inline ColArgs col_args(const Pass& p, int i, int t, const float* x, int64_t ldx) {
  const tt_tower_acts* A = p.A[t];
  const int nchunks = block_chunks(p, i, t);
  return ColArgs{x, ldx, A->pre[i], A->mean[i], A->rstd[i], block_salt(p.P[t], t, i), (int)p.B, p.P[t]->hidden[i], (int)tt_cdiv(p.B, nchunks),
                 nchunks, p.ws[t].col, p.G[t]->bn_b[i], p.G[t]->bn_w[i]};
}
inline BnBwdArgs bn_bwd_args(const Pass& p, int i, int t) {
  const tt_tower_params* P = p.P[t]; const tt_tower_acts* A = p.A[t];
  return BnBwdArgs{d_in(p, i + 1, t), A->pre[i], p.B * P->hidden[i], P->hidden[i], 1.f / (float)p.B, A->mean[i], A->rstd[i], P->bn_w[i],
                   p.G[t]->bn_b[i], p.G[t]->bn_w[i], block_salt(P, t, i)};
}
int check_block_grads(const Pass& p, int i) {
  for (int t = 0; t < p.n; ++t)
    TT_CHECK_ARG(p.G[t]->w[i] && p.G[t]->b[i] && p.G[t]->bn_w[i] && p.G[t]->bn_b[i], "tt_towers_mlp_bwd: NULL gradient buffers of block %d", i);
  return TT_OK;
}
inline GemmNT nt_item(const Pass& p, int t, const float* A, const float* W, const float* bias, float* C, int64_t ldc, int N, int K) {
  GemmNT g{A, K, W, K, bias, C, ldc, p.B, N, K, false, 1.f};
  g.bf16 = p.bf16; g.workspace = p.ws[t].gemm; g.workspace_bytes = p.ws[t].gemm_bytes;
  return g;
}
inline GemmTN tn_item(const Pass& p, int t, int slot, const float* A, int64_t lda, const float* Bm, float* C, int M, int N, float* colsum) {
  GemmTN g{A, lda, Bm, N, C, N, M, N, p.B, p.ws[t].tn[slot], p.ws[t].tn_bytes[slot], colsum};
  g.bf16 = p.bf16;
  return g;
}
int launch_layer_nt(const Pass& p, int i, NtDeferred* defer) {
  GemmNT nt[TT_MAX_SIDES];
  const bool out = i == p.nh;
  for (int t = 0; t < p.n; ++t) {
    const tt_tower_params* P = p.P[t];
    const int N = out ? P->d_out : P->hidden[i];
    nt[t] = nt_item(p, t, layer_in(p, i, t), out ? P->w_out : P->w[i], out ? P->b_out : P->b[i], out ? p.A[t]->y : p.A[t]->pre[i], N, N, in_width(P, i));
    nt[t].a_bf16 = i == 0 && P->x_dtype == TT_BF16;
    nt[t].defer = defer ? &defer[t] : nullptr;
  }
  return tt_gemm_nt_batched(p.st, nt, p.n);
}
int launch_layer_bwd(const Pass& p, int i, TnPending* pend, bool data_grad = true) {
  GemmTN tn[TT_MAX_SIDES]; GemmNN nn[TT_MAX_SIDES];
  const bool out = i == p.nh;
  for (int t = 0; t < p.n; ++t) {
    const tt_tower_params* P = p.P[t]; const tt_tower_grads* g = p.G[t];
    const int M = out ? P->d_out : P->hidden[i], N = in_width(P, i);
    const float* dY = out ? g->d_y : d_in(p, i + 1, t);
    tn[t] = tn_item(p, t, 1 + i, dY, M, layer_in(p, i, t), out ? g->w_out : g->w[i], M, N, out ? g->b_out : g->b[i]);
    tn[t].b_bf16 = i == 0 && P->x_dtype == TT_BF16;
    nn[t] = GemmNN{dY, M, out ? P->w_out : P->w[i], N, d_in(p, i, t), N, p.B, N, M};
    nn[t].bf16 = p.bf16; nn[t].c_bf16 = i == 0 && P->dx_dtype == TT_BF16;
  }
  if (int rc = tt_gemm_tn_batched(p.st, tn, p.n, pend)) return rc;
  return data_grad ? tt_gemm_nn_batched(p.st, nn, p.n) : TT_OK;
}

int sync_hand_out_stats(const Pass& p, const Batch<BnStatArgs>& bs, int hmax) {
  Batch<LocalArgs> la{};
  for (int t = 0; t < p.n; ++t) la.a[t] = LocalArgs{bs.a[t].partial, bs.a[t].nchunks, bs.a[t].H, p.A[t]->bn_sync_local};
  tail_local_stats_kernel<<<dim3((unsigned)tt_cdiv(hmax, 64), (unsigned)p.n), kThreads, 0, p.st>>>(la);
  TT_LAUNCH_CHECK();
  return TT_OK;
}
inline void sync_take_rank_stats(const Pass& p, Batch<BnStatArgs>& bs) {
  for (int t = 0; t < p.n; ++t) {
    bs.a[t].partial = const_cast<float*>(p.A[t]->bn_sync_all); bs.a[t].nchunks = p.P[t]->sync_ranks; bs.a[t].pstride = p.A[t]->bn_sync_stride;
  }
}
int sync_hand_out_colsums(const Pass& p, const Batch<ColArgs>& cols, int gx) {
  Batch<LocalArgs> la{};
  for (int t = 0; t < p.n; ++t) la.a[t] = LocalArgs{cols.a[t].partial, cols.a[t].nchunks, cols.a[t].H, p.G[t]->s_sync_local};
  tail_local_colsum_kernel<<<dim3((unsigned)gx, (unsigned)p.n), kThreads, 0, p.st>>>(la);
  TT_LAUNCH_CHECK();
  return TT_OK;
}
inline float sync_take_rank_colsums(const Pass& p, ColArgs& col, BnBwdArgs& bn, int t, float* raw) {
  const int ranks = p.P[t]->sync_ranks;
  col.partial = const_cast<float*>(p.G[t]->s_sync_all); col.nchunks = ranks; col.pstride = p.G[t]->s_sync_stride;
  bn.invB = 1.f / ((float)p.B * (float)ranks);
  if (raw) { col.out_scale = 1.f / (float)ranks; col.sums_raw = raw; bn.S1 = raw; bn.S2 = raw + col.H; }
  return 1.f / (float)ranks;
}

inline void pack_target(const Pass& p, TailFwdArgs& tf, int t) {
  if (!p.A[t]->emb_packed) return;
  tf.Dp = p.P[t]->d_out <= 32 ? 32 : (p.P[t]->d_out <= 64 ? 64 : 128);
  tf.pk_rows = reinterpret_cast<__bf16*>(p.A[t]->emb_packed);
  tf.pk_frag = tf.pk_rows + tt_cdiv(p.B, 64) * 64 * tf.Dp;
  tf.pk_scale = p.A[t]->emb_pack_scale == 0.f ? 1.f : p.A[t]->emb_pack_scale;
}
inline Batch<TailFwdArgs> tail_fwd_args(const Pass& p, int i, const Batch<BnStatArgs>& bs) {
  Batch<TailFwdArgs> tf{};
  for (int t = 0; t < p.n; ++t) {
    const tt_tower_params* P = p.P[t];
    tf.a[t] = TailFwdArgs{bs.a[t], P->bn_w[i], P->bn_b[i], block_salt(P, t, i), p.A[t]->act[i], P->w_out, P->b_out, P->d_out,
                          p.A[t]->y, p.A[t]->emb, nullptr, nullptr, 0, 1.f};
    pack_target(p, tf.a[t], t);
  }
  return tf;
}
int fwd_narrow_tail(const Pass& p, int i, Batch<BnStatArgs>& bs, const NtDeferred* nd, bool front, const BlockDims& dim) {
  tt_ctx* ctx = p.ctx; hipStream_t st = p.st; const int n = p.n;
  if (p.phase != 2) {
    if (front) {
      Batch<FrontArgs> fb{};
      bool w16 = true;
      for (int t = 0; t < n; ++t) {
        const tt_tower_params* P = p.P[t]; const tt_tower_acts* A = p.A[t];
        const int wx = P->h0 + P->kcat_e;
        fb.a[t] = FrontArgs{A->dense, P->din, P->din, P->w_proj, P->b_proj, P->h0, reinterpret_cast<uint16_t*>(A->x), wx, wx, P->w[i], P->b[i],
                            A->pre[i], bs.a[t], reinterpret_cast<const uint16_t*>(P->w_proj_bf16), reinterpret_cast<const uint16_t*>(P->w_bf16[i])};
        w16 = w16 && P->w_proj_bf16 && P->w_bf16[i] && tt_aligned(P->w_proj_bf16, 16) && tt_aligned(P->w_bf16[i], 16);
      }
      if (w16) {
        TT_LDS_ONCE(kFrontLds, tower_front_kernel<true>);
        tower_front_kernel<true><<<dim3((unsigned)dim.cmax, (unsigned)n), kFrontThreads, kFrontLds, st>>>(fb);
      } else {
        TT_LDS_ONCE(kFrontLds, tower_front_kernel<false>);
        tower_front_kernel<false><<<dim3((unsigned)dim.cmax, (unsigned)n), kFrontThreads, kFrontLds, st>>>(fb);
      }
    } else if (nd[0].splits > 0) {
      Batch<HeadArgs> hb{};
      for (int t = 0; t < n; ++t) hb.a[t] = HeadArgs{nd[t].slabs, nd[t].slab_stride, nd[t].splits, p.P[t]->b[i], p.A[t]->pre[i], bs.a[t]};
      tail_head_kernel<<<dim3((unsigned)dim.cmax, (unsigned)n), kTailThreads, 0, st>>>(hb);
    } else {
      bn_stats_partial_kernel<<<dim3(1, (unsigned)dim.cmax, (unsigned)n), kThreads, 0, st>>>(bs);
    }
    TT_LAUNCH_CHECK();
  }
  if (p.phase == 1) return sync_hand_out_stats(p, bs, dim.hmax);
  if (p.phase == 2) sync_take_rank_stats(p, bs);
  Batch<TailFwdArgs> tf = tail_fwd_args(p, i, bs);
  bool fin = false;
  int mine = 0;
  if (int rc = tt_deferred_host(ctx, TT_DQ_SORT | TT_DQ_COMPACT, st, &mine)) return rc;
  if (mine & TT_DQ_SORT) {
    BnFinishRiders bf{};
    fin = p.phase == 0 && ctx->bn_fin != nullptr;
    for (int t = 0; t < n && fin; ++t) {
      const BnStatArgs& s = bs.a[t];
      bf.r[t] = BnFinishRider{s.partial, s.pstride ? s.pstride : 3 * s.H, s.nchunks, s.H, s.mean, s.rstd, s.rm, s.rv, s.nbt,
                              ctx->bn_fin + t * kBnFinStride};
      tf.a[t].fin = bf.r[t].out;
    }
    if (int rc = tt_keyed_sort_run(ctx->dq->sort, st, &bf, fin ? n : 0)) return rc;
  }
  const int cr_wg = (mine & TT_DQ_COMPACT) ? ctx->dq->compact_wg : 0;
  const int64_t gx = tt_cdiv(p.B, 64) > cr_wg ? tt_cdiv(p.B, 64) : cr_wg;
  const dim3 grid((unsigned)gx, (unsigned)(n + (cr_wg > 0 ? 1 : 0)));
  if (fin) tail_fwd_kernel<true><<<grid, kTailThreads, 0, st>>>(tf, p.drop, p.dropout_p, p.seed, p.seed_dev, ctx->dq->compact, cr_wg);
  else tail_fwd_kernel<false><<<grid, kTailThreads, 0, st>>>(tf, p.drop, p.dropout_p, p.seed, p.seed_dev, ctx->dq->compact, cr_wg);
  tt_deferred_taken(ctx, mine);
  TT_LAUNCH_CHECK();
  return TT_OK;
}
int fwd_wide_tail(const Pass& p, int i, const Batch<BnStatArgs>& bs) {
  tt_ctx* ctx = p.ctx;
  TT_LDS_ONCE(kWideLds, tail_fwd_wide_kernel);
  tail_fwd_wide_kernel<<<dim3((unsigned)tt_cdiv(p.B, 64), (unsigned)p.n), kTailThreads, kWideLds, p.st>>>(tail_fwd_args(p, i, bs), p.drop, p.dropout_p, p.seed, p.seed_dev);
  TT_LAUNCH_CHECK();
  return TT_OK;
}

bool back_items(const Pass& p, GemmBack* gb) {
  if (p.nh < 1 || !p.bf16) return false;
  for (int t = 0; t < p.n; ++t) {
    const tt_tower_params* P = p.P[t]; const tt_tower_grads* g = p.G[t];
    const int wx = P->h0 + P->kcat_e;
    if (P->flags & TT_TOWER_UNFUSED_BACK) return false;
    gb[t] = GemmBack{g->scratch[0], P->hidden[0], p.A[t]->x, wx, wx, P->x_dtype == TT_BF16, p.A[t]->dense, P->din, P->din,
                     P->w[0], P->h0, reinterpret_cast<float*>(g->d_x), wx, P->dx_dtype == TT_BF16, g->w[0], g->b[0],
                     g->w_proj, g->b_proj, p.ws[t].tn[1], p.ws[t].tn_bytes[1], p.ws[t].tn[0], p.ws[t].tn_bytes[0], p.B};
    gb[t].w16 = P->w_bf16[0];
  }
  return tt_gemm_back_supported(gb, p.n);
}
enum LossHost { kLossNobody, kLossTailBwd, kLossGemmBack, kLossTailBwdApply };
int bwd_narrow_tail(const Pass& p, bool back, LossHost* loss) {
  tt_ctx* ctx = p.ctx; hipStream_t st = p.st; const int n = p.n, i = p.nh - 1;
  if (int rc = check_block_grads(p, i)) return rc;
  Batch<ColArgs> cb{}; Batch<TailBwdArgs> tb{}; Batch<TailApplyArgs> tp{};
  for (int t = 0; t < n; ++t) {
    const tt_tower_params* P = p.P[t]; const tt_tower_grads* g = p.G[t];
    const int H = P->hidden[i], D = P->d_out;
    cb.a[t] = col_args(p, i, t, nullptr, 0);
    const int nchunks = cb.a[t].nchunks;
    float* w_slab = reinterpret_cast<float*>((reinterpret_cast<uintptr_t>(p.ws[t].tn[p.nh + 1]) + 255) & ~uintptr_t(255));
    float* b_slab = w_slab + (size_t)nchunks * D * H;
    tb.a[t] = TailBwdArgs{p.A[t]->y, p.A[t]->emb, p.d_emb[t], g->d_y, D, P->w_out, p.A[t]->act[i], d_in(p, p.nh, t), cb.a[t], w_slab, b_slab};
    tp.a[t] = TailApplyArgs{cb.a[t], bn_bwd_args(p, i, t), w_slab, b_slab, D, g->w_out, g->b_out, nchunks, 1.f};
    if (p.phase == 2) tp.a[t].out_scale = sync_take_rank_colsums(p, tp.a[t].col, tp.a[t].bn, t, nullptr);
  }
  int mine = 0;
  if (int rc = tt_deferred_host(ctx, TT_DQ_SCORE_BWD | TT_DQ_LOSS, st, &mine)) return rc;
  bool hosted = false;
  if (mine & TT_DQ_SCORE_BWD) {
    hosted = p.phase == 0 && n == 2 && ctx->dq->score_rows == p.B && ctx->dq->score_dA[0] == p.d_emb[0] && ctx->dq->score_dA[1] == p.d_emb[1];
    for (int t = 0; hosted && t < n; ++t)
      hosted = tb.a[t].D == 64 && tb.a[t].col.H == 64 && tb.a[t].col.rows_per_chunk == 64 && tb.a[t].col.nchunks == (int)tt_cdiv(p.B, 64);
    if (hosted) {
      if (int rc = tt_score_tail_bwd_launch(ctx, tb, p.drop, p.dropout_p, p.seed, p.seed_dev)) return rc;
    } else if (int rc = tt_deferred_flush(ctx, TT_DQ_SCORE_BWD)) {
      return rc;
    }
  }
  *loss = !(mine & TT_DQ_LOSS) ? kLossNobody : hosted ? (back ? kLossGemmBack : kLossTailBwdApply) : p.phase != 2 ? kLossTailBwd : kLossNobody;
  if (p.phase != 2 && !hosted) {
    const int fr_on = *loss == kLossTailBwd;
    tail_bwd_kernel<<<dim3((unsigned)block_dims(p, i).cmax, (unsigned)(n + fr_on)), kTailThreads, 0, st>>>(tb, p.drop, p.dropout_p, p.seed, p.seed_dev, ctx->dq->loss, fr_on);
    tt_deferred_taken(ctx, TT_DQ_LOSS & mine);
    TT_LAUNCH_CHECK();
  }
  if (p.phase == 1) return sync_hand_out_colsums(p, cb, 1);
  const int fr_here = *loss == kLossTailBwdApply;
  tail_bwd_apply_kernel<<<dim3((unsigned)tt_cdiv(p.B, 64), (unsigned)(n + fr_here)), kTailThreads, 0, st>>>(tp, ctx->dq->loss, fr_here);
  if (fr_here) tt_deferred_taken(ctx, TT_DQ_LOSS);
  TT_LAUNCH_CHECK();
  return TT_OK;
}
int bwd_wide_head(const Pass& p, TnPending* pend) {
  const int i = p.nh - 1;
  Batch<TailBwdArgs> tb{};
  for (int t = 0; t < p.n; ++t)
    tb.a[t] = TailBwdArgs{p.A[t]->y, p.A[t]->emb, p.d_emb[t], p.G[t]->d_y, p.P[t]->d_out, p.P[t]->w_out, nullptr, d_in(p, p.nh, t),
                          col_args(p, i, t, nullptr, 0), nullptr, nullptr};
  tail_bwd_wide_kernel<<<dim3((unsigned)block_dims(p, i).cmax, (unsigned)p.n), kWideBwdThreads, 0, p.st>>>(tb, p.drop, p.dropout_p, p.seed, p.seed_dev);
  TT_LAUNCH_CHECK();
  return launch_layer_bwd(p, p.nh, pend, false);
}
int bwd_first_block_back(const Pass& p, const GemmBack* gb, TnPending* pend, bool with_loss) {
  tt_ctx* ctx = p.ctx;
  int mine = 0;
  if (with_loss)
    if (int rc = tt_deferred_host(ctx, TT_DQ_LOSS, p.st, &mine)) return rc;
  if (int rc = tt_gemm_back_batched(p.st, gb, p.n, pend, (mine & TT_DQ_LOSS) ? &ctx->dq->loss : nullptr)) return rc;
  tt_deferred_taken(ctx, mine & TT_DQ_LOSS);
  if (ctx->dq->defer_slabs) return tt_deferred_queue_slabs(ctx, p.st, pend);
  return tt_gemm_tn_flush(p.st, pend);
}

}

extern "C" {

size_t tt_tower_workspace_bytes(const tt_tower_params* p, int64_t B) {
  if (!p || p->n_hidden < 0 || p->n_hidden > TT_MAX_HIDDEN) return 0;
  return ws_layout(p, B, nullptr).total;
}

int tt_towers_mlp_fwd(tt_ctx* ctx, int32_t n, const tt_tower_params* const* P, const tt_tower_acts* const* A, int64_t B,
                      int32_t train, float dropout_p, uint64_t seed, const uint64_t* seed_dev, void* const* workspaces,
                      const size_t* workspace_bytes, tt_stream stream) {
  TT_CHECK_ARG(ctx && A, "tt_towers_mlp_fwd: NULL argument");
  if (int rc = check_batch(n, P, B, dropout_p, workspaces, workspace_bytes, "tt_towers_mlp_fwd")) return rc;
  if (B == 0) return TT_OK;
  for (int t = 0; t < n; ++t)
    TT_CHECK_ARG(A[t] && A[t]->dense && A[t]->x && A[t]->y && A[t]->emb, "tt_towers_mlp_fwd: NULL activation buffers");
  const Pass p = make_pass(ctx, stream, n, P, A, nullptr, nullptr, B, train, dropout_p, seed, seed_dev, workspaces);
  hipStream_t st = p.st;
  if (int rc = check_sync_phase(p, "tt_towers_mlp_fwd")) return rc;
  const int nh = p.nh, phase = p.phase;
  const bool fused = tail_fusable(n, P, train);
  const bool front = fused && front_fusable(n, P, A);
  if (phase != 2 && !front) {
    GemmNT nt[TT_MAX_SIDES];
    for (int t = 0; t < n; ++t) {
      nt[t] = nt_item(p, t, A[t]->dense, P[t]->w_proj, P[t]->b_proj, reinterpret_cast<float*>(A[t]->x), P[t]->h0 + P[t]->kcat_e, P[t]->h0, P[t]->din);
      nt[t].c_bf16 = P[t]->x_dtype == TT_BF16;
    }
    if (int rc = tt_gemm_nt_batched(st, nt, n)) return rc;
  }
  NtDeferred nd[TT_MAX_SIDES];
  for (int i = 0; i < nh; ++i) {
    const bool tail = fused && i == nh - 1;
    Batch<BnStatArgs> bs{}; Batch<BnApplyArgs> ba{};
    for (int t = 0; t < n; ++t) {
      TT_CHECK_ARG(A[t]->pre[i] && A[t]->act[i] && A[t]->mean[i] && A[t]->rstd[i], "tt_towers_mlp_fwd: NULL buffers of block %d", i);
      bs.a[t] = bn_stat_args(p, i, t);
      ba.a[t] = bn_apply_args(p, i, t);
    }
    const BlockDims dim = block_dims(p, i);
    if (phase != 2 && !(front && tail))
      if (int rc = launch_layer_nt(p, i, tail ? nd : nullptr)) return rc;
    if (tail) return fwd_narrow_tail(p, i, bs, nd, front, dim);
    if (train) {
      if (phase != 2) {
        bn_stats_partial_kernel<<<dim3((unsigned)tt_cdiv(dim.hmax, 64), (unsigned)dim.cmax, (unsigned)n), kThreads, 0, st>>>(bs);
        TT_LAUNCH_CHECK();
      }
      if (phase == 1) return sync_hand_out_stats(p, bs, dim.hmax);
      if (phase == 2) sync_take_rank_stats(p, bs);
      if (i == nh - 1 && !fused && wide_tail_ok(n, P, train)) return fwd_wide_tail(p, i, bs);
      bn_stats_finish_kernel<<<dim3((unsigned)tt_cdiv(dim.hmax, 64), (unsigned)n), kThreads, 0, st>>>(bs);
      TT_LAUNCH_CHECK();
    } else {
      bn_eval_prepare_kernel<<<dim3((unsigned)tt_cdiv(dim.hmax, 256), (unsigned)n), 256, 0, st>>>(bs);
      TT_LAUNCH_CHECK();
    }
    bn_apply_kernel<<<dim3((unsigned)ew_grid(ctx, dim.tmax, n), (unsigned)n), kThreads, 0, st>>>(ba, p.drop, dropout_p, seed, seed_dev);
    TT_LAUNCH_CHECK();
  }
  if (int rc = launch_layer_nt(p, nh, nullptr)) return rc;
  Batch<NormArgs> na{};
  for (int t = 0; t < n; ++t) na.a[t] = NormArgs{A[t]->y, nullptr, nullptr, (int)B, P[t]->d_out, A[t]->emb};
  if (!launch_l2norm_fast<false>(st, na, n, B)) l2norm_fwd_kernel<<<dim3((unsigned)tt_cdiv(B, 4), (unsigned)n), kThreads, 0, st>>>(na);
  TT_LAUNCH_CHECK();
  for (int t = 0; t < n; ++t)
    if (A[t]->emb_packed)
      if (int rc = tt_score_pack_bf16(ctx, A[t]->emb, B, P[t]->d_out, A[t]->emb_pack_scale, A[t]->emb_packed, stream)) return rc;
  return TT_OK;
}

int tt_towers_mlp_bwd(tt_ctx* ctx, int32_t n, const tt_tower_params* const* P, const tt_tower_acts* const* A,
                      const float* const* d_emb, const tt_tower_grads* const* G, int64_t B, int32_t train, float dropout_p,
                      uint64_t seed, const uint64_t* seed_dev, void* const* workspaces, const size_t* workspace_bytes,
                      tt_stream stream) {
  TT_CHECK_ARG(ctx && A && G && d_emb, "tt_towers_mlp_bwd: NULL argument");
  if (int rc = check_batch(n, P, B, dropout_p, workspaces, workspace_bytes, "tt_towers_mlp_bwd")) return rc;
  TT_CHECK_ARG(B >= 1, "tt_towers_mlp_bwd: B < 1");
  for (int t = 0; t < n; ++t) {
    const tt_tower_grads* g = G[t];
    TT_CHECK_ARG(A[t] && g && d_emb[t] && g->w_proj && g->b_proj && g->w_out && g->b_out && g->d_x && g->d_y,
                 "tt_towers_mlp_bwd: NULL gradient buffers");
  }
  const Pass p = make_pass(ctx, stream, n, P, A, G, d_emb, B, train, dropout_p, seed, seed_dev, workspaces);
  hipStream_t st = p.st;
  const int nh = p.nh, phase = p.phase;
  const bool fused = tail_fusable(n, P, train);
  const bool wide = !fused && wide_tail_ok(n, P, train);
  if (int rc = check_sync_phase(p, "tt_towers_mlp_bwd")) return rc;
  if (!(fused && phase == 0))
    if (int rc = tt_deferred_flush(ctx, TT_DQ_SCORE_BWD)) return rc;
  if (!fused && !wide && phase != 2) {
    Batch<NormArgs> na{};
    for (int t = 0; t < n; ++t) na.a[t] = NormArgs{A[t]->y, A[t]->emb, d_emb[t], (int)B, P[t]->d_out, G[t]->d_y};
    if (!launch_l2norm_fast<true>(st, na, n, B)) l2norm_bwd_kernel<<<dim3((unsigned)tt_cdiv(B, 4), (unsigned)n), kThreads, 0, st>>>(na);
    TT_LAUNCH_CHECK();
  }
  for (int t = 0; t < n; ++t) TT_CHECK_ARG(d_in(p, nh, t), "tt_towers_mlp_bwd: NULL scratch buffer");
  TnPending pend;
  GemmBack gb[TT_MAX_SIDES];
  const bool back = back_items(p, gb);
  LossHost loss = kLossNobody;
  if (fused) {
    if (int rc = bwd_narrow_tail(p, back, &loss)) return rc;
    if (phase == 1) return TT_OK;
  } else if (wide) {
    if (phase != 2)
      if (int rc = bwd_wide_head(p, &pend)) return rc;
  } else if (phase != 2) {
    if (int rc = launch_layer_bwd(p, nh, &pend)) return rc;
  }
  for (int i = nh - 1; i >= 0; --i) {
    const bool last = i == nh - 1;
    if (int rc = check_block_grads(p, i)) return rc;
    Batch<ColArgs> cb{}; Batch<BnBwdArgs> bb{};
    for (int t = 0; t < n; ++t) {
      cb.a[t] = col_args(p, i, t, d_in(p, i + 1, t), P[t]->hidden[i]);
      bb.a[t] = bn_bwd_args(p, i, t);
    }
    const BlockDims dim = block_dims(p, i);
    if (wide && last && phase != 1) {
      Batch<TailApplyArgs> tp{};
      for (int t = 0; t < n; ++t) {
        tp.a[t] = TailApplyArgs{cb.a[t], bb.a[t], nullptr, nullptr, P[t]->d_out, nullptr, nullptr, 0, 1.f};
        if (phase == 2) tp.a[t].out_scale = sync_take_rank_colsums(p, tp.a[t].col, tp.a[t].bn, t, nullptr);
      }
      tail_bwd_apply_wide_kernel<<<dim3((unsigned)tt_cdiv(B, 64), (unsigned)n), kTailThreads, 0, st>>>(tp);
      TT_LAUNCH_CHECK();
    } else if (!(fused && last)) {
      if (phase != 2 && !(wide && last)) {
        colsum_partial_kernel<<<dim3((unsigned)tt_cdiv(dim.hmax, 64), (unsigned)dim.cmax, (unsigned)n), kThreads, 0, st>>>(cb, p.drop, dropout_p, seed, seed_dev);
        TT_LAUNCH_CHECK();
      }
      if (phase == 1) {
        if (int rc = tt_gemm_tn_flush(st, &pend)) return rc;
        return sync_hand_out_colsums(p, cb, (int)tt_cdiv(dim.hmax, 64));
      }
      if (phase == 2)
        for (int t = 0; t < n; ++t)
          sync_take_rank_colsums(p, cb.a[t], bb.a[t], t, p.ws[t].col + 2 * (size_t)dim.hmax * kMaxChunks);
      colsum_finish_kernel<<<dim3((unsigned)tt_cdiv(dim.hmax, 64), (unsigned)n), kThreads, 0, st>>>(cb);
      TT_LAUNCH_CHECK();
      bn_bwd_apply_kernel<<<dim3((unsigned)ew_grid(ctx, dim.tmax, n), (unsigned)n), kThreads, 0, st>>>(bb, p.train, p.drop, dropout_p, seed, seed_dev);
      TT_LAUNCH_CHECK();
    }
    for (int t = 0; t < n; ++t) TT_CHECK_ARG(d_in(p, i, t), "tt_towers_mlp_bwd: NULL scratch buffer");
    if (i == 0 && back) return bwd_first_block_back(p, gb, &pend, loss == kLossGemmBack);
    if (int rc = launch_layer_bwd(p, i, &pend)) return rc;
  }
  GemmTN tn[TT_MAX_SIDES];
  for (int t = 0; t < n; ++t) {
    tn[t] = tn_item(p, t, 0, reinterpret_cast<const float*>(G[t]->d_x), P[t]->h0 + P[t]->kcat_e, A[t]->dense, G[t]->w_proj, P[t]->h0, P[t]->din,
                    G[t]->b_proj);
    tn[t].a_bf16 = P[t]->dx_dtype == TT_BF16;
  }
  if (int rc = tt_gemm_tn_batched(st, tn, n, &pend)) return rc;
  return tt_gemm_tn_flush(st, &pend);
}

int tt_tower_mlp_fwd(tt_ctx* ctx, const tt_tower_params* p, const tt_tower_acts* a, int64_t B, int32_t train, float dropout_p,
                     uint64_t seed, const uint64_t* seed_dev, void* workspace, size_t workspace_bytes, tt_stream stream) {
  return tt_towers_mlp_fwd(ctx, 1, &p, &a, B, train, dropout_p, seed, seed_dev, &workspace, &workspace_bytes, stream);
}

int tt_tower_mlp_bwd(tt_ctx* ctx, const tt_tower_params* p, const tt_tower_acts* a, const float* d_emb, const tt_tower_grads* g,
                     int64_t B, int32_t train, float dropout_p, uint64_t seed, const uint64_t* seed_dev, void* workspace,
                     size_t workspace_bytes, tt_stream stream) {
  return tt_towers_mlp_bwd(ctx, 1, &p, &a, &d_emb, &g, B, train, dropout_p, seed, seed_dev, &workspace, &workspace_bytes, stream);
}

int tt_linear_fwd(tt_ctx* ctx, const float* X, int64_t ldx, const float* W, const float* bias, float* Y, int64_t ldy, int64_t M,
                  int32_t N, int32_t K, int32_t relu, tt_stream stream) {
  TT_CHECK_ARG(ctx && (M == 0 || (X && W && Y)), "tt_linear_fwd: NULL argument");
  TT_CHECK_ARG(M >= 0 && N >= 1 && K >= 1 && ldx >= K && ldy >= N, "tt_linear_fwd: bad shape");
  TT_CHECK_ARG(M < ((int64_t)1 << 31), "tt_linear_fwd: M too large");
  return tt_gemm_nt(reinterpret_cast<hipStream_t>(stream), X, ldx, W, K, bias, Y, ldy, M, N, K, relu != 0);
}

}

#ifdef TT_TAIL_STAMPS
extern "C" int tt_debug_tail_stamps(int which, unsigned long long* host_out ) {
  return hipMemcpyFromSymbol(host_out, HIP_SYMBOL(g_tail_stamps), sizeof(unsigned long long) * 512 * 8,
                             sizeof(unsigned long long) * 512 * 8 * (size_t)which, hipMemcpyDeviceToHost) == hipSuccess ? 0 : -2;
}
#endif
```

jodalrob-twotower_amd/ops.py:

```python
from __future__ import annotations

import ctypes as C
from dataclasses import dataclass
from typing import List, Optional, Sequence

import torch

from . import _lib as L
from .config import settings
from ._lib import TT_BF16, TT_F32, TT_GRAD_DENSE_ACC, TT_GRAD_DENSE_SET, TT_GRAD_SPARSE


class KernelTimer:

    def __init__(self, names=None):
        self.names = set(names) if names else None
        self.records = {}

    def wants(self, name):
        return self.names is None or name in self.names

    def summary(self):
        torch.cuda.synchronize()
        return {n: (len(ev), sum(a.elapsed_time(b) for a, b in ev) / max(len(ev), 1)) for n, ev in self.records.items()}
# ... 233 lines not shown
        return
    ws, E = plan.grad_ws
    dev = out.device
    with _timed("tt_embed_grad_finish"):
        L.check(L.load().tt_embed_grad_finish(L.ctx(dev), E, L.ptr(plan.seg_offsets), plan.M, L.ptr(out), L.ptr(ws), ws.numel(),
                                              L.stream(dev)), "tt_embed_grad_finish")
    plan.finish_deferred = None


def adam_dense(p, g, m, v, step, lr, b1, b2, eps, wd, hp_dev=None):
    dev = p.device
    with _timed("tt_adam_dense_step"):
        L.check(L.load().tt_adam_dense_step(L.ctx(dev), L.ptr(p), L.ptr(g), L.ptr(m), L.ptr(v), p.numel(), step, lr, b1, b2,
                                            eps, wd, L.ptr(hp_dev), L.stream(dev)), "tt_adam_dense_step")


def _adam_tensors(items):
    arr = (L.AdamTensor * len(items))()
    for i, (p, g, m, v) in enumerate(items):
        arr[i] = L.AdamTensor(p.data_ptr(), g.data_ptr(), m.data_ptr(), v.data_ptr(), p.numel())
    return arr


def _fused_step(who, entry, head, plan: "DedupPlan", grad_rows, tail):
    fin = ()
    if plan.finish_deferred is not None:
        if plan.finish_deferred.data_ptr() != grad_rows.data_ptr():
            raise RuntimeError(f"{who}: the plan's deferred gradient is not the one handed to the optimiser")
        ws = plan.grad_ws[0]
        fin = (L.ptr(plan.seg_offsets), L.ptr(ws), ws.numel())
    name = entry + "_finish" if fin else entry
    with _timed(entry):
        L.check(getattr(L.load(), name)(*head, *fin, *tail), name)
    plan.finish_deferred = None


def adam_multi(items, step, lr, b1, b2, eps, wd, hp_dev=None):
    if not items:
        return
    dev = items[0][0].device
    with _timed("tt_adam_multi_step"):
        L.check(L.load().tt_adam_multi_step(L.ctx(dev), _adam_tensors(items), len(items), step, lr, b1, b2, eps, wd, L.ptr(hp_dev),
                                            L.stream(dev)), "tt_adam_multi_step")


def adam_sparse(table, m, v, plan: DedupPlan, grad_rows, step, lr, b1, b2, eps, wd, hp_dev=None):
    dev = table.device
    embed_grad_finish(plan)
    with _timed("tt_sparse_adam_step"):
        L.check(L.load().tt_sparse_adam_step(L.ctx(dev), L.ptr(table), L.ptr(m), L.ptr(v), table.shape[0], table.shape[1],
                                             L.ptr(plan.unique_rows), L.ptr(grad_rows), L.ptr(plan.n_unique), plan.M, step,
                                             lr, b1, b2, eps, wd, L.ptr(hp_dev), L.stream(dev)), "tt_sparse_adam_step")


def adam_fused(items, table, m, v, plan: DedupPlan, grad_rows, step, lr, b1, b2, eps, wd, hp_dev=None):
    dev = table.device
    head = (L.ctx(dev), _adam_tensors(items), len(items), L.ptr(table), L.ptr(m), L.ptr(v), table.shape[0], table.shape[1],
            L.ptr(plan.unique_rows), L.ptr(grad_rows), L.ptr(plan.n_unique), plan.M)
    tail = (step, lr, b1, b2, eps, wd, L.ptr(hp_dev), L.stream(dev))
    _fused_step("adam_fused", "tt_adam_fused_step", head, plan, grad_rows, tail)


def rowwise_adagrad_sparse(table, acc, plan: DedupPlan, grad_rows, lr, eps, wd, hp_dev=None):
    dev = table.device
    embed_grad_finish(plan)
    with _timed("tt_rowwise_adagrad_sparse_step"):
        L.check(L.load().tt_rowwise_adagrad_sparse_step(L.ctx(dev), L.ptr(table), L.ptr(acc), table.shape[0], table.shape[1],
                                                        L.ptr(plan.unique_rows), L.ptr(grad_rows), L.ptr(plan.n_unique), plan.M,
                                                        lr, eps, wd, L.ptr(hp_dev), L.stream(dev)), "tt_rowwise_adagrad_sparse_step")


def rowwise_adagrad_dense(table, acc, grad, lr, eps, wd, hp_dev=None):
    dev = table.device
    with _timed("tt_rowwise_adagrad_dense_step"):
        L.check(L.load().tt_rowwise_adagrad_dense_step(L.ctx(dev), L.ptr(table), L.ptr(acc), L.ptr(grad), table.shape[0], table.shape[1],
                                                       lr, eps, wd, L.ptr(hp_dev), L.stream(dev)), "tt_rowwise_adagrad_dense_step")


def adam_rowwise_adagrad_fused(items, step, lr, b1, b2, eps, wd, hp_dev, table, acc, plan: DedupPlan, grad_rows, t_lr, t_eps, t_wd,
                               t_hp_dev=None):
    dev = table.device
    head = (L.ctx(dev), _adam_tensors(items), len(items), step, lr, b1, b2, eps, wd, L.ptr(hp_dev), L.ptr(table), L.ptr(acc),
            table.shape[0], table.shape[1], L.ptr(plan.unique_rows), L.ptr(grad_rows), L.ptr(plan.n_unique), plan.M)
    tail = (t_lr, t_eps, t_wd, L.ptr(t_hp_dev), L.stream(dev))
    _fused_step("adam_rowwise_adagrad_fused", "tt_adam_rowwise_adagrad_fused_step", head, plan, grad_rows, tail)


def _fill(arr, tensors):
    for i, t in enumerate(tensors):
        arr[i] = t.data_ptr() if t is not None else 0


def tower_params_struct(din, h0, kcat_e, hidden, d_out, w_proj, b_proj, ws, bs, bn_w, bn_b, bn_rm, bn_rv, w_out, b_out,
                        bn_nbt=(), compute_dtype=TT_F32, x_dtype=TT_F32, dx_dtype=TT_F32, flags=0, w_proj_bf16=None, w_bf16=()):
    if len(hidden) > L.TT_MAX_HIDDEN:
        raise ValueError(f"at most {L.TT_MAX_HIDDEN} hidden blocks per tower are supported")
    p = L.TowerParams()
    p.din, p.h0, p.kcat_e, p.n_hidden, p.d_out = din, h0, kcat_e, len(hidden), d_out
    for i, h in enumerate(hidden):
        p.hidden[i] = h
    p.w_proj, p.b_proj, p.w_out, p.b_out = w_proj.data_ptr(), b_proj.data_ptr(), w_out.data_ptr(), b_out.data_ptr()
    _fill(p.w, ws); _fill(p.b, bs); _fill(p.bn_w, bn_w); _fill(p.bn_b, bn_b); _fill(p.bn_rm, bn_rm); _fill(p.bn_rv, bn_rv)
    _fill(p.bn_nbt, bn_nbt)
    p.compute_dtype, p.x_dtype, p.dx_dtype, p.flags = compute_dtype, x_dtype, dx_dtype, flags
    p.w_proj_bf16 = w_proj_bf16.data_ptr() if w_proj_bf16 is not None else 0
    _fill(p.w_bf16, w_bf16)
    return p


def adam_hparams(step, lr, b1, b2, eps, wd):
    out = (L.f32 * 6)()
    L.load().tt_adam_hparams(step, lr, b1, b2, eps, wd, C.byref(out))
    return list(out)


def tower_workspace(params, B, dev):
    nb = L.load().tt_tower_workspace_bytes(C.byref(params), B)
    return L.workspace(dev, nb)


def tower_fwd(params, acts, B, train, p_drop, seed, dev, seed_dev=None):
    ws = tower_workspace(params, B, dev)
    with _timed("tt_tower_mlp_fwd"):
        L.check(L.load().tt_tower_mlp_fwd(L.ctx(dev), C.byref(params), C.byref(acts), B, int(train), p_drop, seed, L.ptr(seed_dev), L.ptr(ws),
                                          ws.numel(), L.stream(dev)), "tt_tower_mlp_fwd")


def tower_bwd(params, acts, d_emb, grads, B, train, p_drop, seed, dev, seed_dev=None):
    ws = tower_workspace(params, B, dev)
    with _timed("tt_tower_mlp_bwd"):
        L.check(L.load().tt_tower_mlp_bwd(L.ctx(dev), C.byref(params), C.byref(acts), L.ptr(d_emb), C.byref(grads), B,
                                          int(train), p_drop, seed, L.ptr(seed_dev), L.ptr(ws), ws.numel(), L.stream(dev)), "tt_tower_mlp_bwd")


def _tower_workspaces(params_list, B, dev):
    lib = L.load()
    sizes = [(lib.tt_tower_workspace_bytes(C.byref(p), B) + 255) // 256 * 256 for p in params_list]
    buf = L.workspace(dev, sum(sizes))
    ptrs, off = (L.vp * len(sizes))(), 0
    for i, z in enumerate(sizes):
        ptrs[i] = buf.data_ptr() + off
        off += z
    return buf, ptrs, (L.sz * len(sizes))(*sizes)


def towers_fwd(params_list, acts_list, B, train, p_drop, seed, dev, seed_dev=None):
    n = len(params_list)
    _, wptrs, wsizes = _tower_workspaces(params_list, B, dev)
    P = (C.POINTER(L.TowerParams) * n)(*[C.pointer(p) for p in params_list])
    A = (C.POINTER(L.TowerActs) * n)(*[C.pointer(a) for a in acts_list])
    with _timed("tt_towers_mlp_fwd"):
        L.check(L.load().tt_towers_mlp_fwd(L.ctx(dev), n, P, A, B, int(train), p_drop, seed, L.ptr(seed_dev), wptrs, wsizes,
                                           L.stream(dev)), "tt_towers_mlp_fwd")


def towers_bwd(params_list, acts_list, d_embs, grads_list, B, train, p_drop, seed, dev, seed_dev=None):
    n = len(params_list)
    _, wptrs, wsizes = _tower_workspaces(params_list, B, dev)
    P = (C.POINTER(L.TowerParams) * n)(*[C.pointer(p) for p in params_list])
    A = (C.POINTER(L.TowerActs) * n)(*[C.pointer(a) for a in acts_list])
    G = (C.POINTER(L.TowerGrads) * n)(*[C.pointer(g) for g in grads_list])
    D = (L.vp * n)(*[d.data_ptr() for d in d_embs])
    with _timed("tt_towers_mlp_bwd"):
        L.check(L.load().tt_towers_mlp_bwd(L.ctx(dev), n, P, A, D, G, B, int(train), p_drop, seed, L.ptr(seed_dev), wptrs, wsizes,
                                           L.stream(dev)), "tt_towers_mlp_bwd")


LQ_MAX_TWO_INV_T = 40.0


def _lq_vec(lq, B, dev, name):
    if not isinstance(lq, torch.Tensor):
        raise TypeError(f"{name} must be a torch.Tensor, got {type(lq).__name__}")
    if lq.dtype != torch.float32:
        raise TypeError(f"{name} must be float32, got {lq.dtype}")
    if lq.dim() != 1 or lq.shape[0] != B:
        raise ValueError(f"{name} must have shape [{B}], got {list(lq.shape)}")
    if lq.device != dev:
        raise ValueError(f"{name} is on {lq.device}, the scores on {dev}")
    return lq.contiguous()


def _lq_check_t(inv_t):
    if 2.0 * abs(inv_t) > LQ_MAX_TWO_INV_T:
        raise ValueError(f"logQ correction needs 2/T <= {LQ_MAX_TWO_INV_T:g} (T >= 0.05), got 1/T = {inv_t:g}")


def _lq_pair(a, b, Ra, Rb, dev, names):
    return () if a is None else (_lq_vec(a, Ra, dev, names[0]), _lq_vec(b, Rb, dev, names[1]))


def _ent_vec(e, B, dev, name):
    if not isinstance(e, torch.Tensor):
        raise TypeError(f"{name} must be a torch.Tensor, got {type(e).__name__}")
    if e.dtype != torch.int32:
        raise TypeError(f"{name} must be int32, got {e.dtype}")
    if e.dim() != 1 or e.shape[0] != B:
        raise ValueError(f"{name} must have shape [{B}], got {list(e.shape)}")
    if e.device != dev:
        raise ValueError(f"{name} is on {e.device}, the scores on {dev}")
    return e


def score_mask_ids(ent_n, ent_c, B, dev):
    Bp = (B + 63) // 64 * 64
    if B == Bp and ent_n is not None and ent_c is not None:
        en, ec = _ent_vec(ent_n, B, dev, "ent_n"), _ent_vec(ent_c, B, dev, "ent_c")
        if en.is_contiguous() and ec.is_contiguous() and en.data_ptr() % 16 == 0 and ec.data_ptr() % 16 == 0:
            return en, ec
    out = torch.zeros((2, Bp), dtype=torch.int32, device=dev)
    for k, (e, name) in enumerate(((ent_n, "ent_n"), (ent_c, "ent_c"))):
        if e is None:
            out[k, :B] = torch.arange(B, dtype=torch.int32, device=dev)
        else:
            out[k, :B] = _ent_vec(e, B, dev, name)
    return out[0], out[1]


def _mask_args(ent, lq, n_lq):
    return (L.ptr(ent[0]), L.ptr(ent[1])) + (tuple(map(L.ptr, lq)) if lq else (None,) * n_lq)


def score_pair_weights(w, B, dev):
    if not isinstance(w, torch.Tensor):
        raise TypeError(f"pair_weight must be a torch.Tensor, got {type(w).__name__}")
    if w.dtype != torch.float32:
        raise TypeError(f"pair_weight must be float32, got {w.dtype}")
    if w.dim() != 1 or w.shape[0] != B:
        raise ValueError(f"pair_weight must have shape [{B}], got {list(w.shape)}")
    if w.device != torch.device(dev):
        raise ValueError(f"pair_weight is on {w.device}, the scores on {dev}")
    w = w.contiguous()
    g = torch.empty((B + 63) // 64 * 64, dtype=torch.float32, device=w.device)
    with _timed("tt_score_prepare_pw"):
        L.check(L.load().tt_score_prepare_pw(L.ctx(w.device), L.ptr(w), B, L.ptr(g), L.stream(w.device)), "tt_score_prepare_pw")
    return g


def _pw_args(pw, ent, lq, n_lq):
    return (L.ptr(pw),) + ((L.ptr(ent[0]), L.ptr(ent[1])) if ent is not None else (None, None)) \
        + (tuple(map(L.ptr, lq)) if lq else (None,) * n_lq)


def score_dir_fwd(A, Bm, inv_t, shift, diag_offset=0, want_sumscore=True, lq_b=None, ent=None):
    dev, Ra, Rb, D = A.device, A.shape[0], Bm.shape[0], A.shape[1]
    lq = () if lq_b is None else (_lq_vec(lq_b, Rb, dev, "lq_b"),)
    f = torch.empty((3, Ra), dtype=torch.float32, device=dev)
    rank = torch.empty(Ra, dtype=torch.int32, device=dev)
    if ent is not None:
        name = "tt_score_dir_fwd_mask"
        with _timed(name):
            L.check(getattr(L.load(), name)(L.ctx(dev), L.ptr(A), L.ptr(Bm), Ra, Rb, D, inv_t, shift, diag_offset, *_mask_args(ent, lq, 1),
                                            L.ptr(f[0]), L.ptr(f[1]), L.ptr(rank), L.ptr(f[2]) if want_sumscore else None, L.stream(dev)),
                    name)
        return f[0], f[1], rank, f[2]
    name = "tt_score_dir_fwd_lq" if lq else "tt_score_dir_fwd"
    with _timed(name):
        L.check(getattr(L.load(), name)(L.ctx(dev), L.ptr(A), L.ptr(Bm), Ra, Rb, D, inv_t, shift, diag_offset, *map(L.ptr, lq),
                                        L.ptr(f[0]), L.ptr(f[1]), L.ptr(rank), L.ptr(f[2]) if want_sumscore else None, L.stream(dev)),
                name)
    return f[0], f[1], rank, f[2]


def score_loss_finish(B, shift, rowsum, colsum, diag, row_rank, col_rank, sumscore, lq_n=None, lq_c=None, pw=None):
    dev = rowsum.device
    lq = _lq_pair(lq_n, lq_c, B, B, dev, ("lq_n", "lq_c"))
    out = torch.empty(8, dtype=torch.float32, device=dev)
    loss = torch.empty((), dtype=torch.float32, device=dev)
    if pw is not None:
        name = "tt_score_loss_finish_pw"
        with _timed(name):
            L.check(getattr(L.load(), name)(L.ctx(dev), B, shift, L.ptr(pw), *(map(L.ptr, lq) if lq else (None, None)), L.ptr(rowsum),
                                            L.ptr(colsum), L.ptr(diag), L.ptr(row_rank), L.ptr(col_rank), L.ptr(sumscore), L.ptr(out),
                                            L.ptr(loss), L.stream(dev)), name)
        return out, loss
    name = "tt_score_loss_finish_lq" if lq else "tt_score_loss_finish"
    with _timed(name):
        L.check(getattr(L.load(), name)(L.ctx(dev), B, shift, *map(L.ptr, lq), L.ptr(rowsum), L.ptr(colsum), L.ptr(diag),
                                        L.ptr(row_rank), L.ptr(col_rank), L.ptr(sumscore), L.ptr(out), L.ptr(loss), L.stream(dev)),
                name)
    return out, loss


def score_dir_bwd(A, Bm, inv_t, shift, diag_offset, sumexp_a, sumexp_b, d_loss, scale, lq_a=None, lq_b=None, ent=None, pw=None):
    dev, Ra, Rb, D = A.device, A.shape[0], Bm.shape[0], A.shape[1]
    lq = _lq_pair(lq_a, lq_b, Ra, Rb, dev, ("lq_a", "lq_b"))
    dA = torch.empty_like(A)
    if pw is not None:
        name = "tt_score_dir_bwd_pw"
        with _timed(name):
            L.check(getattr(L.load(), name)(L.ctx(dev), L.ptr(A), L.ptr(Bm), Ra, Rb, D, inv_t, shift, diag_offset, *_pw_args(pw, ent, lq, 2),
                                            L.ptr(sumexp_a), L.ptr(sumexp_b), L.ptr(d_loss), scale, L.ptr(dA), L.stream(dev)), name)
        return dA
    if ent is not None:
        name = "tt_score_dir_bwd_mask"
        with _timed(name):
            L.check(getattr(L.load(), name)(L.ctx(dev), L.ptr(A), L.ptr(Bm), Ra, Rb, D, inv_t, shift, diag_offset, *_mask_args(ent, lq, 2),
                                            L.ptr(sumexp_a), L.ptr(sumexp_b), L.ptr(d_loss), scale, L.ptr(dA), L.stream(dev)), name)
        return dA
    name = "tt_score_dir_bwd_lq" if lq else "tt_score_dir_bwd"
    with _timed(name):
        L.check(getattr(L.load(), name)(L.ctx(dev), L.ptr(A), L.ptr(Bm), Ra, Rb, D, inv_t, shift, diag_offset, *map(L.ptr, lq),
                                        L.ptr(sumexp_a), L.ptr(sumexp_b), L.ptr(d_loss), scale, L.ptr(dA), L.stream(dev)), name)
    return dA


# ... 550 lines not shown
```

jodalrob-twotower_amd/towers.py:

```python
from __future__ import annotations

import ctypes as C
from typing import Dict, List, Optional, Sequence

import torch
from ._lib import no_dynamo as _no_dynamo
import torch.nn as nn

from . import _lib as L
from . import ops
from .config import settings
from .cat_embed import CategoricalEmbedder, EmbeddingStore


_DEBUG_KEEP = None


def _sync_comm(sides):
    if not sides:
        return None
    comms = [getattr(s.tower, "sync_comm", None) for s in sides]
    if any(c is None for c in comms) or not all(s.train for s in sides):
        return None
    if len({s.B for s in sides}) != 1 or len({s.p_drop for s in sides}) != 1:
        raise ValueError("SyncBN needs one batch size and one dropout rate for all towers of a pass")
    return comms[0]


def _al(n: int) -> int:
    return (n + 63) // 64 * 64


def _run_pass(items, one, many, key, sync):
    sides = [it[0] for it in items]
    comm = _sync_comm(sides)
    if comm is None and not (len(sides) > 1 and len({(s.B, s.tower.n_hidden) + key(s) for s in sides}) == 1):
        for s, *args in items:
            one(s.tower._params(), *args, s.B, s.train, s.p_drop, s.seed, s.emb.device, s.tower._seed_dev)
        return None
    s0 = sides[0]
    params = [s.tower._params() for s in sides]
    args = [list(col) for col in zip(*(it[1:] for it in items))]
    call = lambda: many(params, *args, s0.B, s0.train, s0.p_drop, s0.seed, s0.emb.device, s0.tower._seed_dev)
    keep = None
    if comm is None:
        call()
    else:
        at, local, gathered, stride, per = sync
        widths = [per * s.tower.tower_hidden_dims[1] for s in sides]
        loc = torch.empty(sum(widths), dtype=torch.float32, device=s0.emb.device)
        where = [(it[at], p, 4 * sum(widths[:k])) for k, (it, p) in enumerate(zip(items, params))]
        for s, (holder, p, off) in zip(sides, where):
            setattr(holder, local, loc.data_ptr() + off)
            p.sync_phase, p.sync_ranks, p.rng_row_offset = 1, comm.world, comm.rank * s.B
        try:
            call()
            allg = comm.all_gather(loc)
            for holder, p, off in where:
                setattr(holder, gathered, allg.data_ptr() + off)
                setattr(holder, stride, loc.numel())
                p.sync_phase = 2
            call()
        finally:
            for p in params:
                p.sync_phase = 0
        keep = (loc, allg)
    for s in sides:
        s.seed = s0.seed
    return keep


class BaseTower(nn.Module):
    def __init__(self, categorical_keys: List[str], metadata_path: str = "meta/metadata.csv", table_name: str = "notice",
                 categorical_embedding_dim: int = 64, dense_input_dim: int = 256,
                 tower_hidden_dims: Optional[List[int]] = None, final_embedding_dim: int = 128, dropout_rate: float = 0.2,
                 device="cuda:0", embedding_grad: Optional[str] = None, materialize_tables: bool = True,
                 mlp_dtype: Optional[str] = None):
        super().__init__()
        if tower_hidden_dims is None:
            tower_hidden_dims = [256, 128]
        self.mlp_dtype = mlp_dtype or settings.mlp_dtype
        if self.mlp_dtype not in ("fp32", "bf16"):
            raise ValueError(f"mlp_dtype must be 'fp32' or 'bf16', got {self.mlp_dtype!r}")
        io = settings.tower_io_dtype if self.mlp_dtype == "bf16" else "none"
        if io not in ("none", "x", "dx", "both"):
            raise ValueError(f"settings.tower_io_dtype must be none|x|dx|both, got {io!r}")
        self.x_dtype = torch.bfloat16 if io in ("x", "both") else torch.float32
        self.dx_dtype = torch.bfloat16 if io in ("dx", "both") else torch.float32
        self.unfused_tail, self.unfused_front, self.unfused_back = settings.tower_unfused_tail, settings.tower_unfused_front, settings.tower_unfused_back
        self.categorical_keys = list(categorical_keys)
        self.exchange = None
        self.sync_comm = None
        self.pack_for_score = False
        self._last_packed = None
        self.pack_scale = 1.0
        self._seed_dev = None
        self._w16 = None
        self._seed_override = None
        self.device = device
        self.tower_hidden_dims = list(tower_hidden_dims)
        self.final_embedding_dim = final_embedding_dim
        self.dropout_rate = float(dropout_rate)
        self.dense_input_dim = dense_input_dim
        dev = torch.device(device)
        self.categorical_embedder = CategoricalEmbedder(keys=self.categorical_keys, metadata_path=metadata_path,
                                                        table_name=table_name, embedding_dim=categorical_embedding_dim,
                                                        device=str(dev), embedding_grad=embedding_grad,
                                                        materialize=materialize_tables)
        self.dense_projection = nn.Linear(dense_input_dim, tower_hidden_dims[0])
        self._build_mlp(categorical_embedding_dim, tower_hidden_dims, final_embedding_dim, dropout_rate)
        self._struct_key = None
        self._params_struct = None
        self.to(dev)

    def _build_mlp(self, categorical_embedding_dim, tower_hidden_dims, final_embedding_dim, dropout_rate):
        in_dim = tower_hidden_dims[0] + len(self.categorical_keys) * categorical_embedding_dim
        layers = []
        for h in tower_hidden_dims[1:]:
            layers += [nn.Linear(in_dim, h), nn.ReLU(), nn.BatchNorm1d(h), nn.Dropout(dropout_rate)]
            in_dim = h
        layers.append(nn.Linear(in_dim, final_embedding_dim))
        self.mlp = nn.Sequential(*layers)

    @property
    def n_hidden(self) -> int:
        return len(self.tower_hidden_dims) - 1

    def dense_parameters(self) -> List[torch.Tensor]:
        ps = [self.dense_projection.weight, self.dense_projection.bias]
        for i in range(self.n_hidden):
            lin, bn = self.mlp[4 * i], self.mlp[4 * i + 2]
            ps += [lin.weight, lin.bias, bn.weight, bn.bias]
        ps += [self.mlp[4 * self.n_hidden].weight, self.mlp[4 * self.n_hidden].bias]
        return ps

    def _params(self):
        nh = self.n_hidden
        lins = [self.mlp[4 * i] for i in range(nh)]
        bns = [self.mlp[4 * i + 2] for i in range(nh)]
        out = self.mlp[4 * nh]
        tensors = [self.dense_projection.weight, self.dense_projection.bias, out.weight, out.bias]
        for lin, bn in zip(lins, bns):
            tensors += [lin.weight, lin.bias, bn.weight, bn.bias, bn.running_mean, bn.running_var]
        w16 = self._w16
        key = tuple(t.data_ptr() for t in tensors) + tuple(b.num_batches_tracked.data_ptr() for b in bns) + (self.mlp_dtype, self.x_dtype, self.dx_dtype, self.unfused_tail, self.unfused_front, self.unfused_back) + \
            ((w16[0].data_ptr(),) + tuple(w.data_ptr() for w in w16[1]) if w16 is not None else ())
        if key != self._struct_key:
            for t in tensors:
                if t.dtype != torch.float32 or not t.is_contiguous():
                    raise TypeError("tower parameters must be contiguous float32")
            E = self.categorical_embedder.embedding_dim
            self._params_struct = ops.tower_params_struct(
                self.dense_input_dim, self.tower_hidden_dims[0], len(self.categorical_keys) * E, self.tower_hidden_dims[1:],
                self.final_embedding_dim, self.dense_projection.weight, self.dense_projection.bias,
                [l.weight for l in lins], [l.bias for l in lins], [b.weight for b in bns], [b.bias for b in bns],
                [b.running_mean for b in bns], [b.running_var for b in bns], out.weight, out.bias,
                bn_nbt=[b.num_batches_tracked for b in bns],
                compute_dtype=ops.TT_BF16 if self.mlp_dtype == "bf16" else ops.TT_F32,
                x_dtype=ops.TT_BF16 if self.x_dtype == torch.bfloat16 else ops.TT_F32,
                dx_dtype=ops.TT_BF16 if self.dx_dtype == torch.bfloat16 else ops.TT_F32,
                flags=(ops.L.TT_TOWER_UNFUSED_TAIL if self.unfused_tail else 0) | (ops.L.TT_TOWER_UNFUSED_FRONT if self.unfused_front else 0) | (ops.L.TT_TOWER_UNFUSED_BACK if self.unfused_back else 0),
                w_proj_bf16=None if w16 is None else w16[0], w_bf16=() if w16 is None else w16[1])
            self._struct_key = key
        return self._params_struct

    @property
    def x_width(self) -> int:
        return self.tower_hidden_dims[0] + len(self.categorical_keys) * self.categorical_embedder.embedding_dim

    @_no_dynamo
    def forward(self, tower_input: Dict[str, torch.Tensor]) -> torch.Tensor:
        return run_towers([self], [tower_input])[0]


class NoticeTower(BaseTower):
    def __init__(self, categorical_keys: List[str], metadata_path: str = "meta/metadata.csv",
                 categorical_embedding_dim: int = 64, dense_input_dim: int = 256,
                 tower_hidden_dims: Optional[List[int]] = None, final_embedding_dim: int = 128, dropout_rate: float = 0.2,
                 device="cuda:0", embedding_grad: Optional[str] = None, materialize_tables: bool = True,
                 mlp_dtype: Optional[str] = None):
        super().__init__(categorical_keys=categorical_keys, metadata_path=metadata_path, table_name="notice",
                         categorical_embedding_dim=categorical_embedding_dim, dense_input_dim=dense_input_dim,
                         tower_hidden_dims=tower_hidden_dims, final_embedding_dim=final_embedding_dim,
                         dropout_rate=dropout_rate, device=device, embedding_grad=embedding_grad,
                         materialize_tables=materialize_tables, mlp_dtype=mlp_dtype)


class CompanyTower(BaseTower):
    def __init__(self, categorical_keys: List[str], metadata_path: str = "meta/metadata.csv",
                 categorical_embedding_dim: int = 64, dense_input_dim: int = 128,
                 tower_hidden_dims: Optional[List[int]] = None, final_embedding_dim: int = 128, dropout_rate: float = 0.2,
                 device="cuda:0", embedding_grad: Optional[str] = None, materialize_tables: bool = True,
                 mlp_dtype: Optional[str] = None):
        super().__init__(categorical_keys=categorical_keys, metadata_path=metadata_path, table_name="company",
                         categorical_embedding_dim=categorical_embedding_dim, dense_input_dim=dense_input_dim,
                         tower_hidden_dims=tower_hidden_dims, final_embedding_dim=final_embedding_dim,
                         dropout_rate=dropout_rate, device=device, embedding_grad=embedding_grad,
                         materialize_tables=materialize_tables, mlp_dtype=mlp_dtype)


def run_towers(towers: Sequence[BaseTower], inputs: Sequence[Dict]) -> List[torch.Tensor]:
    flat = []
    for tw, inp in zip(towers, inputs):
        dev = tw.categorical_embedder.store.device
        dense = inp["dense"].to(dev)
        kjt = inp["kjt"]
        values = (kjt.to(dev) if hasattr(kjt, "to") else kjt).values()
        flat += [dense, values] + tw.dense_parameters() + tw.categorical_embedder.table_parameters()
    outs = _TowersFn.apply(tuple(towers), *flat)
    outs = list(outs) if isinstance(outs, tuple) else [outs]
    for tw, o in zip(towers, outs):
        if tw._last_packed is not None:
            o._tt_packed, tw._last_packed = tw._last_packed, None
    return outs


class _Side:
    __slots__ = ("tower", "B", "acts", "acts_struct", "buf", "x", "emb", "train", "seed", "p_drop", "sync_keep", "packed", "values")


class _TowersFn(torch.autograd.Function):
    @staticmethod
    def forward(ctx, towers, *flat):
        sides: List[_Side] = []
        pos = 0
        grad_on = any(ctx.needs_input_grad)
        spans = []
        lookups: Dict[int, list] = {}
        for tw in towers:
            emb = tw.categorical_embedder
            nd, nt = len(tw.dense_parameters()), len(emb.table_parameters())
            dense, values = flat[pos], flat[pos + 1]
            spans.append((pos, nd, nt))
            pos += 2 + nd + nt
            dev = emb.store.device
            if dense.dim() != 2 or dense.shape[1] != tw.dense_input_dim:
                raise ValueError(f"dense input must be [B, {tw.dense_input_dim}], got {tuple(dense.shape)}")
            dense = dense.to(dtype=torch.float32).contiguous()
            values = values.to(dtype=torch.int64).contiguous()
            B, K, E = dense.shape[0], len(emb.keys), emb.embedding_dim
            if values.numel() != B * K:
                raise ValueError(f"kjt carries {values.numel()} ids but the batch needs B*K = {B}*{K}")
            s = _Side()
            s.tower, s.B, s.train = tw, B, tw.training
            s.p_drop = tw.dropout_rate if tw.training else 0.0
            s.seed = 0 if s.p_drop <= 0 else (tw._seed_override if tw._seed_override is not None else
                                              int(torch.empty((), dtype=torch.int64).random_().item()))
            s.values = values
            s.acts = (dense,)
            sides.append(s)
        pre = {}
        if towers[0].exchange is None and grad_on:
            by_store: Dict[int, list] = {}
            for s in sides:
                emb = s.tower.categorical_embedder
                if s.B and len(emb.keys):
                    by_store.setdefault(id(emb.store), []).append(s)
            for group in by_store.values():
                st = group[0].tower.categorical_embedder.store
                xs = st.x_for([g.values for g in group], [(g.B, g.tower.x_width, g.tower.x_dtype) for g in group])
                if xs is not None:
                    for g, x in zip(group, xs):
                        pre[id(g)] = x
        for s in sides:
            tw, B, dense, values = s.tower, s.B, s.acts[0], s.values
            emb = tw.categorical_embedder
            K, E = len(emb.keys), emb.embedding_dim
            dev = emb.store.device
            hid = tw.tower_hidden_dims[1:]
            px = pre.get(id(s))
            x_f32 = tw.x_dtype == torch.float32 and px is None
            sizes = [_al(B * tw.x_width) if x_f32 else 0] + [_al(B * h) for h in hid for _ in (0, 1)] + \
                    [_al(h) for h in hid for _ in (0, 1)] + [_al(B * tw.final_embedding_dim)]
            s.buf = torch.empty(sum(sizes), dtype=torch.float32, device=dev)
            offs = [0]
            for z in sizes:
                offs.append(offs[-1] + z)
            s.x = px if px is not None else (s.buf[:B * tw.x_width].view(B, tw.x_width) if x_f32 else
                                             torch.empty((B, tw.x_width), dtype=tw.x_dtype, device=dev))
            s.emb = torch.empty((B, tw.final_embedding_dim), dtype=torch.float32, device=dev)
            a = L.TowerActs()
            base, esz = s.buf.data_ptr(), 4
            a.dense, a.x, a.emb = dense.data_ptr(), s.x.data_ptr(), s.emb.data_ptr()
            nh = len(hid)
            for i in range(nh):
                a.pre[i] = base + esz * offs[1 + 2 * i]
                a.act[i] = base + esz * offs[2 + 2 * i]
                a.mean[i] = base + esz * offs[1 + 2 * nh + 2 * i]
                a.rstd[i] = base + esz * offs[2 + 2 * nh + 2 * i]
            a.y = base + esz * offs[1 + 4 * nh]
            s.packed = None
            if tw.pack_for_score and B:
                s.packed = torch.empty(L.load().tt_score_pack_bytes(B, tw.final_embedding_dim), dtype=torch.uint8, device=dev)
                a.emb_packed, a.emb_pack_scale = s.packed.data_ptr(), float(tw.pack_scale)
            s.acts_struct = a
            if K and B:
                lookups.setdefault(id(emb.store), []).append((s, emb.lookup_side(values, s.x[:, tw.tower_hidden_dims[0]:]), px is not None))
        plans = []
        exch = towers[0].exchange
        ctx.exch, ctx.exch_state = exch, None
        if exch is not None:
            group = [g for grp in lookups.values() for g in grp]
            if group:
                ctx.exch_state = exch.forward([g[1] for g in group], group[0][0].B, grad_on)
                ctx.exch_sides = [g[0] for g in group]
            lookups = {}
        for group in lookups.values():
            store: EmbeddingStore = group[0][0].tower.categorical_embedder.store
            B = group[0][0].B
            if any(g[0].B != B for g in group):
                for g in group:
                    rows = ops.embed_lookup(store.weight, [g[1]], g[0].B, want_rows=grad_on)
                    plans.append([store, [g[0]], ops.dedup_plan(rows, store.rows) if grad_on else None])
                continue
            km = store.rows_km_for([g[1].ids for g in group]) if (grad_on and 0 < B <= ops.KEYED_MAX_B) else None
            sm = store.rows_sm_for([g[1].ids for g in group]) if km is not None else None
            if all(g[2] for g in group) and km is not None:
                rows = None
            elif sm is not None and store.weight.shape[1] % 4 == 0 and all(g[1].out.stride(0) % 4 == 0 for g in group):
                rows = None
                ops.embed_lookup_rows(store.weight, sm, [g[1] for g in group], B)
            else:
                rows = ops.embed_lookup(store.weight, [g[1] for g in group], B, want_rows=grad_on and km is None)
            plans.append([store, [g[0] for g in group], None, rows if km is None else km, grad_on, km is not None])
        for pl in plans:
            if len(pl) == 6:
                store, psides, _, rows, want_plan, key_major = pl
                plan = None
                if want_plan:
                    Bs = psides[0].B
                    if 0 < Bs <= ops.KEYED_MAX_B:
                        plan = ops.dedup_plan_keyed(rows, [len(q.tower.categorical_embedder.keys) for q in psides], Bs, key_major,
                                                    E=int(store.E))
                    else:
                        plan = ops.dedup_plan(rows, store.rows)
                    plan.keep = rows
                pl[:] = [store, psides, plan]
        live = [s for s in sides if s.B]
        keep = _run_pass([(s, s.acts_struct) for s in live], ops.tower_fwd, ops.towers_fwd, lambda s: (s.train, s.p_drop),
                         (1, "bn_sync_local", "bn_sync_all", "bn_sync_stride", 3))
        for s in live if keep else ():
            s.sync_keep = keep
        for s in sides:
            s.tower._last_packed = None if s.packed is None else (s.packed, float(s.tower.pack_scale))
        ctx.sides, ctx.plans, ctx.spans, ctx.n_flat = sides, plans, spans, len(flat)
        outs = tuple(s.emb.view(s.emb.shape) for s in sides)
        ctx.mark_non_differentiable(*[o for o, s in zip(outs, sides) if s.B == 0])
        return outs

    @staticmethod
    def backward(ctx, *d_embs):
        grads = [None] * ctx.n_flat
        dxs = {}
        exch = ctx.exch
        if exch is not None and exch.world > 1:
            d_embs = [None if d is None else d * (1.0 / exch.world) for d in d_embs]
        flat_grads = []
        work = [(s, d, sp) for s, d, sp in zip(ctx.sides, d_embs, ctx.spans) if s.B and d is not None]
        prepared = []
        side_sizes = []
        for s, _, _ in work:
            tw = s.tower
            side_sizes.append(([_al(p.numel()) for p in tw.dense_parameters()],
                               [_al(s.B * tw.x_width) if tw.dx_dtype == torch.float32 else 0] +
                               [_al(s.B * h) for h in tw.tower_hidden_dims[1:]] + [_al(s.B * tw.final_embedding_dim)]))
        dense_total = sum(sum(d) for d, _ in side_sizes)
        buf = torch.empty(dense_total + sum(sum(r) for _, r in side_sizes), dtype=torch.float32, device=work[0][0].emb.device) if work else None
        dense_at, scratch_at = 0, dense_total
        for (s, d_emb, (pos, nd, nt)), (dsz, rsz) in zip(work, side_sizes):
            tw = s.tower
            dev = s.emb.device
            d_emb = d_emb.to(dtype=torch.float32).contiguous()
            dps = tw.dense_parameters()
            hid = tw.tower_hidden_dims[1:]
            B = s.B
            dx_f32 = tw.dx_dtype == torch.float32
            offs = [dense_at]
            for z in dsz[:-1]:
                offs.append(offs[-1] + z)
            dense_at += sum(dsz)
            offs.append(scratch_at)
            for z in rsz:
                offs.append(offs[-1] + z)
            scratch_at += sum(rsz)
            base = buf.data_ptr()
            views = [buf[offs[i]:offs[i] + p.numel()].view(p.shape) for i, p in enumerate(dps)]
            g = L.TowerGrads()
            g.w_proj, g.b_proj = base + 4 * offs[0], base + 4 * offs[1]
            for i in range(len(hid)):
                g.w[i], g.b[i] = base + 4 * offs[2 + 4 * i], base + 4 * offs[3 + 4 * i]
                g.bn_w[i], g.bn_b[i] = base + 4 * offs[4 + 4 * i], base + 4 * offs[5 + 4 * i]
                g.scratch[i] = base + 4 * offs[len(dps) + 1 + i]
            g.w_out, g.b_out = base + 4 * offs[len(dps) - 2], base + 4 * offs[len(dps) - 1]
            d_x = buf[offs[len(dps)]:offs[len(dps)] + B * tw.x_width].view(B, tw.x_width) if dx_f32 else \
                torch.empty((B, tw.x_width), dtype=tw.dx_dtype, device=dev)
            g.d_x = d_x.data_ptr()
            g.d_y = base + 4 * offs[len(dps) + 1 + len(hid)]
            prepared.append((s, d_emb, g))
            if _DEBUG_KEEP is not None:
                _DEBUG_KEEP.append({"buf": buf, "offs": offs, "n_dense": len(dps), "hidden": hid, "B": B, "acts": s.buf, "emb": s.emb,
                                    "d_emb": d_emb})
            for i, v in enumerate(views):
                grads[pos + 2 + i] = v
            dxs[id(s)] = d_x[:, tw.tower_hidden_dims[0]:]
        _run_pass([(s, s.acts_struct, d, g) for s, d, g in prepared], ops.tower_bwd, ops.towers_bwd, lambda s: (s.train, s.p_drop, s.seed),
                  (3, "s_sync_local", "s_sync_all", "s_sync_stride", 2))
        if exch is not None:
            if ctx.exch_state is not None:
                srcs = []
                for s in ctx.exch_sides:
                    K = len(s.tower.categorical_embedder.keys)
                    d = dxs.get(id(s))
                    if d is None:
                        d = torch.zeros((s.B, K * exch.E), dtype=s.tower.dx_dtype, device=s.emb.device)
                    srcs.append((d, K))
                exch.backward(ctx.exch_state, srcs, ctx.exch_sides[0].B)
            if buf is not None and dense_total:
                flat_grads.append(buf[:dense_total])
                L.flush_deferred(buf.device)
            exch.all_reduce_dense(flat_grads)
        for store, plan_sides, plan in ctx.plans:
            if plan is None:
                continue
            srcs = []
            for s in plan_sides:
                K = len(s.tower.categorical_embedder.keys)
                d = dxs.get(id(s))
                if d is None:
                    d = torch.zeros((s.B, K * store.E), dtype=s.tower.dx_dtype, device=store.device)
                srcs.append((d, K))
            store.accumulate_grad(plan, srcs, plan_sides[0].B)
        return (None, *grads)


def tower_dense_param_names(n_hidden: int) -> List[str]:
    names = ["dense_projection.weight", "dense_projection.bias"]
    for i in range(n_hidden):
        names += [f"mlp.{4 * i}.weight", f"mlp.{4 * i}.bias", f"mlp.{4 * i + 2}.weight", f"mlp.{4 * i + 2}.bias"]
    names += [f"mlp.{4 * n_hidden}.weight", f"mlp.{4 * n_hidden}.bias"]
    return names
```

Measured before the change: 37.90 million.

## Fuse embedding-row gather into the tower front kernel

Adds a GATHER variant of the fused front kernel. It reads embedding table rows directly through per-chunk row indices staged in LDS, converts them to bf16 for the GEMM operand and writes x for backward. The separate embed_lookup_rows launch and its round trip of x through HBM are skipped when the pass qualifies (single store, w16 weights, power-of-two E, no sync). In exchange it adds LDS use, index staging with an extra barrier per row block, and narrower per-thread float4 gathers inside the GEMM pipeline.

```diff
diff --git a/include/twotower.h b/include/twotower.h
--- a/include/twotower.h
+++ b/include/twotower.h
@@ -191,6 +191,7 @@
 #define TT_TOWER_UNFUSED_TAIL 1
 #define TT_TOWER_UNFUSED_FRONT 2
 #define TT_TOWER_UNFUSED_BACK 4
+#define TT_TOWER_UNFUSED_GATHER 8
 
 typedef struct tt_tower_acts {
   const float* dense;
@@ -206,6 +207,10 @@
   float* bn_sync_local;
   const float* bn_sync_all;
   int64_t bn_sync_stride;
+  const float* gather_table;
+  const int32_t* gather_rows;
+  int32_t gather_K;
+  int32_t gather_E;
 } tt_tower_acts;
 
 typedef struct tt_tower_grads {
@@ -237,6 +242,7 @@
 int tt_towers_mlp_fwd(tt_ctx* ctx, int32_t n, const tt_tower_params* const* p, const tt_tower_acts* const* a,
                       int64_t B, int32_t train, float dropout_p, uint64_t seed, const uint64_t* seed_dev,
                       void* const* workspaces, const size_t* workspace_bytes, tt_stream stream);
+int tt_towers_fwd_gathers(int32_t n, const tt_tower_params* const* p, const tt_tower_acts* const* a, int64_t B, int32_t train);
 int tt_towers_mlp_bwd(tt_ctx* ctx, int32_t n, const tt_tower_params* const* p, const tt_tower_acts* const* a,
                       const float* const* d_emb, const tt_tower_grads* const* g, int64_t B, int32_t train,
                       float dropout_p, uint64_t seed, const uint64_t* seed_dev, void* const* workspaces,
diff --git a/jodalrob-twotower_amd/_lib.py b/jodalrob-twotower_amd/_lib.py
--- a/jodalrob-twotower_amd/_lib.py
+++ b/jodalrob-twotower_amd/_lib.py
@@ -15,6 +15,7 @@
 TT_TOWER_UNFUSED_TAIL = 1
 TT_TOWER_UNFUSED_FRONT = 2
 TT_TOWER_UNFUSED_BACK = 4
+TT_TOWER_UNFUSED_GATHER = 8
 TT_GRAD_SHORT_SEGMENTS = 0x100
 TT_GRAD_PLANNED = 0x200
 TT_GRAD_DEFER_FINISH = 0x400
@@ -81,7 +82,8 @@
 
 class TowerActs(C.Structure):
     _fields_ = [("dense", vp), ("x", vp), ("pre", _H), ("act", _H), ("mean", _H), ("rstd", _H), ("y", vp), ("emb", vp), ("emb_packed", vp), ("emb_pack_scale", f32),
-                ("bn_sync_local", vp), ("bn_sync_all", vp), ("bn_sync_stride", i64)]
+                ("bn_sync_local", vp), ("bn_sync_all", vp), ("bn_sync_stride", i64),
+                ("gather_table", vp), ("gather_rows", vp), ("gather_K", i32), ("gather_E", i32)]
 
 
 class TowerGrads(C.Structure):
@@ -135,6 +137,7 @@
                                    f32, u64, vp, vp, sz, vp]),
     "tt_towers_mlp_fwd": (C.c_int, [vp, i32, C.POINTER(C.POINTER(TowerParams)), C.POINTER(C.POINTER(TowerActs)), i64, i32, f32, u64,
                                     vp, C.POINTER(vp), C.POINTER(sz), vp]),
+    "tt_towers_fwd_gathers": (C.c_int, [i32, C.POINTER(C.POINTER(TowerParams)), C.POINTER(C.POINTER(TowerActs)), i64, i32]),
     "tt_towers_mlp_bwd": (C.c_int, [vp, i32, C.POINTER(C.POINTER(TowerParams)), C.POINTER(C.POINTER(TowerActs)), C.POINTER(vp),
                                     C.POINTER(C.POINTER(TowerGrads)), i64, i32, f32, u64, vp, C.POINTER(vp), C.POINTER(sz), vp]),
     "tt_score_dir_fwd": (C.c_int, [vp, vp, vp, i64, i64, i32, f32, f32, i64, vp, vp, vp, vp, vp]),
diff --git a/jodalrob-twotower_amd/config.py b/jodalrob-twotower_amd/config.py
--- a/jodalrob-twotower_amd/config.py
+++ b/jodalrob-twotower_amd/config.py
@@ -19,6 +19,7 @@
     graph_weight_shadows: bool = True
     graph_ingest_rows: bool = True
     graph_ingest_lookup: bool = False
+    front_gather: bool = True
     grad_planned: bool = True
 
     @classmethod
diff --git a/jodalrob-twotower_amd/csrc/tt_tower.hip b/jodalrob-twotower_amd/csrc/tt_tower.hip
--- a/jodalrob-twotower_amd/csrc/tt_tower.hip
+++ b/jodalrob-twotower_amd/csrc/tt_tower.hip
@@ -393,11 +393,13 @@
   const float* w; const float* bias; float* pre;
   BnStatArgs s;
   const uint16_t* w_proj16; const uint16_t* w16;
+  const float* table; const int32_t* rows; int K, E;
 };
 constexpr int kFS = 136;
 constexpr int kFrontThreads = 512;
 constexpr int kFrontA = 64 * kFS * 2, kFrontB = 128 * kFS * 2;
 constexpr int kFrontLds = 2 * kFrontA + 2 * kFrontB + kFrontA + 4 * 64 * 12;
+constexpr int kFrontLdsMax = 160 * 1024;
 
 using tl_bf16x4 = __attribute__((ext_vector_type(4))) __bf16;
 __device__ __forceinline__ void front_put4(__bf16* dst, const float4& v, bool live) {
@@ -412,7 +414,7 @@
   return *reinterpret_cast<const T*>(reinterpret_cast<const char*>(base) + off);
 }
 
-template <bool W16>
+template <bool W16, bool GATHER = false>
 __global__ __launch_bounds__(kFrontThreads) void tower_front_kernel(Batch<FrontArgs> batch) {
   const FrontArgs& f = batch.a[blockIdx.y];
   const BnStatArgs& a = f.s;
@@ -424,6 +426,7 @@
   __bf16* Pt = reinterpret_cast<__bf16*>(front_smem + 2 * kFrontA + 2 * kFrontB);
   Wf (*sh)[64] = reinterpret_cast<Wf (*)[64]>(front_smem + 3 * kFrontA + 2 * kFrontB);
   float* part = reinterpret_cast<float*>(bufB);
+  int32_t* idxs = reinterpret_cast<int32_t*>(front_smem + kFrontLds);
   const int t = threadIdx.x, lane = t & 63, wave = t >> 6, li = lane & 31, lh = lane >> 5;
   const int c = t & 63, rq = t >> 6;
   const int r0 = blockIdx.x * a.rows_per_chunk, r1 = min(B, r0 + a.rows_per_chunk);
@@ -435,7 +438,20 @@
   const int pn = (wave >> 1) * 32 + li;
   const float bp = pn < h0 ? f.b_proj[pn] : 0.f;
   float x0 = 0.f, s = 0.f, q = 0.f, cnt = 0.f;
+  const int gK = GATHER ? f.K : 0, gE = GATHER ? f.E : 8, gsh = __builtin_ctz(gE), gke = kx - h0;
+  auto gather_src = [&](int st, int ps) -> const float4* {
+    const int kr = 128 * st + xk - h0;
+    const int kk = (kr >= 0 && kr < gke) ? kr : (xk & (gE - 1));
+    const int64_t row = idxs[(xrow + 32 * ps) * gK + (kk >> gsh)];
+    return reinterpret_cast<const float4*>(f.table + row * gE + (kk & (gE - 1)));
+  };
   for (int b0 = r0; b0 < r1; b0 += 64) {
+    int32_t gi[4];
+    if (GATHER) {
+      const int64_t g0 = (int64_t)b0 * gK, glast = (int64_t)B * gK - 1;
+#pragma unroll
+      for (int j = 0; j < 4; ++j) gi[j] = f.rows[min(g0 + min(t + 512 * j, 64 * gK - 1), glast)];
+    }
     constexpr int NPB = W16 ? 4 : 8, NQB = W16 ? 2 : 4;
     float4 pa[2][4], pb[2][NPB];
     uint32_t oa[4], ob[NPB];
@@ -454,8 +470,16 @@
       for (int ps = 0; ps < NPB; ++ps) pb[st][ps] = W16 ? front_ld<float4>(f.w_proj16, ob[ps] + ko16) : front_ld<float4>(f.w_proj, ob[ps] + ko);
     }
     uint4 qa[3][2];
+    float4 qg[3][2][2];
     float4 qb[3][NQB];
     uint32_t ox[2], ow[NQB];
+    if (GATHER) {
+#pragma unroll
+      for (int j = 0; j < 4; ++j)
+        if (t + 512 * j < 64 * gK) idxs[t + 512 * j] = gi[j];
+      for (int i = t + 2048; i < 64 * gK; i += 512) idxs[i] = f.rows[min((int64_t)b0 * gK + i, (int64_t)B * gK - 1)];
+      __syncthreads();
+    }
 #pragma unroll
     for (int ps = 0; ps < 2; ++ps) ox[ps] = (uint32_t)(min(b0 + xrow + 32 * ps, B - 1) * (int)f.ldx + xkb) * 2u;
 #pragma unroll
@@ -465,7 +489,17 @@
     for (int u = 0; u < 2; ++u) {
       const int ka = 128 * u + xk, kb = 128 * u + fk;
 #pragma unroll
-      for (int ps = 0; ps < 2; ++ps) qa[u][ps] = front_ld<uint4>(f.x, ox[ps] + (ka < kx ? 256u * u : 0u));
+      for (int ps = 0; ps < 2; ++ps) {
+        if (GATHER) {
+          qg[u][ps][0] = qg[u][ps][1] = float4{0.f, 0.f, 0.f, 0.f};
+          if (128 * u + 128 > h0) {
+            const float4* src = gather_src(u, ps);
+            qg[u][ps][0] = src[0]; qg[u][ps][1] = src[1];
+          }
+        } else {
+          qa[u][ps] = front_ld<uint4>(f.x, ox[ps] + (ka < kx ? 256u * u : 0u));
+        }
+      }
 #pragma unroll
       for (int ps = 0; ps < NQB; ++ps)
         qb[u][ps] = W16 ? front_ld<float4>(f.w16, ow[ps] + (ka < kx ? 256u * u : 0u)) : front_ld<float4>(f.w, ow[ps] + (kb < kx ? 512u * u : 0u));
@@ -490,7 +524,14 @@
       {
         const int ka = 256 + xk, kb = 256 + fk;
 #pragma unroll
-        for (int ps = 0; ps < 2; ++ps) qa[2][ps] = front_ld<uint4>(f.x, ox[ps] + (ka < kx ? 512u : 0u));
+        for (int ps = 0; ps < 2; ++ps) {
+          if (GATHER) {
+            const float4* src = gather_src(2, ps);
+            qg[2][ps][0] = src[0]; qg[2][ps][1] = src[1];
+          } else {
+            qa[2][ps] = front_ld<uint4>(f.x, ox[ps] + (ka < kx ? 512u : 0u));
+          }
+        }
 #pragma unroll
         for (int ps = 0; ps < NQB; ++ps)
           qb[2][ps] = W16 ? front_ld<float4>(f.w16, ow[ps] + (ka < kx ? 512u : 0u)) : front_ld<float4>(f.w, ow[ps] + (kb < kx ? 1024u : 0u));
@@ -534,8 +575,22 @@
           __bf16* A = bufA + (st & 1) * 64 * kFS;
           __bf16* Bm = bufB + (st & 1) * 128 * kFS;
 #pragma unroll
-          for (int ps = 0; ps < 2; ++ps)
-            *reinterpret_cast<uint4*>(A + (xrow + 32 * ps) * kFS + xk) = (128 * st + xk < kx) ? qa[u][ps] : uint4{0u, 0u, 0u, 0u};
+          for (int ps = 0; ps < 2; ++ps) {
+            if (GATHER) {
+              const float4 lo = qg[u][ps][0], hi = qg[u][ps][1];
+              const bool live = 128 * st + xk >= h0 && 128 * st + xk < kx;
+              uint4 o;
+              o.x = (uint32_t)tt_f2bf(lo.x) | ((uint32_t)tt_f2bf(lo.y) << 16);
+              o.y = (uint32_t)tt_f2bf(lo.z) | ((uint32_t)tt_f2bf(lo.w) << 16);
+              o.z = (uint32_t)tt_f2bf(hi.x) | ((uint32_t)tt_f2bf(hi.y) << 16);
+              o.w = (uint32_t)tt_f2bf(hi.z) | ((uint32_t)tt_f2bf(hi.w) << 16);
+              *reinterpret_cast<uint4*>(A + (xrow + 32 * ps) * kFS + xk) = live ? o : uint4{0u, 0u, 0u, 0u};
+              if (live && b0 + xrow + 32 * ps < r1)
+                *reinterpret_cast<uint4*>(f.x + (int64_t)(b0 + xrow + 32 * ps) * f.ldx + 128 * st + xk) = o;
+            } else {
+              *reinterpret_cast<uint4*>(A + (xrow + 32 * ps) * kFS + xk) = (128 * st + xk < kx) ? qa[u][ps] : uint4{0u, 0u, 0u, 0u};
+            }
+          }
 #pragma unroll
           for (int ps = 0; ps < NQB; ++ps) {
             if (W16) *reinterpret_cast<float4*>(Bm + (xrow + 32 * ps) * kFS + xk) = (128 * st + xk < kx) ? qb[u][ps] : float4{0.f, 0.f, 0.f, 0.f};
@@ -545,7 +600,14 @@
           {
             const int ka = 128 * (st + 3) + xk, kb = 128 * (st + 3) + fk;
 #pragma unroll
-            for (int ps = 0; ps < 2; ++ps) qa[u][ps] = front_ld<uint4>(f.x, ox[ps] + (ka < kx ? 256u * (uint32_t)(st + 3) : 0u));
+            for (int ps = 0; ps < 2; ++ps) {
+              if (GATHER) {
+                const float4* src = gather_src(st + 3, ps);
+                qg[u][ps][0] = src[0]; qg[u][ps][1] = src[1];
+              } else {
+                qa[u][ps] = front_ld<uint4>(f.x, ox[ps] + (ka < kx ? 256u * (uint32_t)(st + 3) : 0u));
+              }
+            }
 #pragma unroll
             for (int ps = 0; ps < NQB; ++ps)
               qb[u][ps] = W16 ? front_ld<float4>(f.w16, ow[ps] + (ka < kx ? 256u * (uint32_t)(st + 3) : 0u))
@@ -1344,6 +1406,22 @@
   }
   return true;
 }
+inline bool front_w16(const tt_tower_params* p) {
+  return p->w_proj_bf16 && p->w_bf16[0] && tt_aligned(p->w_proj_bf16, 16) && tt_aligned(p->w_bf16[0], 16);
+}
+inline bool wants_gather(const tt_tower_acts* a) { return a->gather_table || a->gather_rows || a->gather_K || a->gather_E; }
+inline bool front_gathers(int n, const tt_tower_params* const* P, const tt_tower_acts* const* A, int64_t B, int train) {
+  if (B < 1 || !tail_fusable(n, P, train) || !front_fusable(n, P, A)) return false;
+  for (int t = 0; t < n; ++t) {
+    const tt_tower_params* p = P[t]; const tt_tower_acts* a = A[t];
+    if (p->sync_phase != 0 || (p->flags & TT_TOWER_UNFUSED_GATHER) || !front_w16(p)) return false;
+    if (!a->gather_table || !a->gather_rows || !tt_aligned(a->gather_table, 16) || !tt_aligned(a->gather_rows, 4)) return false;
+    const int K = a->gather_K, E = a->gather_E;
+    if (K < 1 || E < 8 || E > 256 || (E & (E - 1)) != 0 || (int64_t)K * E != p->kcat_e) return false;
+    if (kFrontLds + 64 * (int64_t)K * (int64_t)sizeof(int32_t) > kFrontLdsMax) return false;
+  }
+  return true;
+}
 inline bool wide_tail_ok(int n, const tt_tower_params* const* P, int train) {
   if (!train || P[0]->compute_dtype != TT_BF16) return false;
   for (int t = 0; t < n; ++t) {
@@ -1584,20 +1662,27 @@
   }
   return tf;
 }
-int fwd_narrow_tail(const Pass& p, int i, Batch<BnStatArgs>& bs, const NtDeferred* nd, bool front, const BlockDims& dim) {
+int fwd_narrow_tail(const Pass& p, int i, Batch<BnStatArgs>& bs, const NtDeferred* nd, bool front, bool gather, const BlockDims& dim) {
   tt_ctx* ctx = p.ctx; hipStream_t st = p.st; const int n = p.n;
   if (p.phase != 2) {
     if (front) {
       Batch<FrontArgs> fb{};
       bool w16 = true;
+      int kmax = 0;
       for (int t = 0; t < n; ++t) {
         const tt_tower_params* P = p.P[t]; const tt_tower_acts* A = p.A[t];
         const int wx = P->h0 + P->kcat_e;
         fb.a[t] = FrontArgs{A->dense, P->din, P->din, P->w_proj, P->b_proj, P->h0, reinterpret_cast<uint16_t*>(A->x), wx, wx, P->w[i], P->b[i],
-                            A->pre[i], bs.a[t], reinterpret_cast<const uint16_t*>(P->w_proj_bf16), reinterpret_cast<const uint16_t*>(P->w_bf16[i])};
-        w16 = w16 && P->w_proj_bf16 && P->w_bf16[i] && tt_aligned(P->w_proj_bf16, 16) && tt_aligned(P->w_bf16[i], 16);
-      }
-      if (w16) {
+                            A->pre[i], bs.a[t], reinterpret_cast<const uint16_t*>(P->w_proj_bf16), reinterpret_cast<const uint16_t*>(P->w_bf16[i]),
+                            A->gather_table, A->gather_rows, A->gather_K, A->gather_E};
+        w16 = w16 && front_w16(P);
+        kmax = A->gather_K > kmax ? A->gather_K : kmax;
+      }
+      if (gather) {
+        const int lds = kFrontLds + 64 * kmax * (int)sizeof(int32_t);
+        TT_LDS_ONCE(kFrontLdsMax, tower_front_kernel<true, true>);
+        tower_front_kernel<true, true><<<dim3((unsigned)dim.cmax, (unsigned)n), kFrontThreads, lds, st>>>(fb);
+      } else if (w16) {
         TT_LDS_ONCE(kFrontLds, tower_front_kernel<true>);
         tower_front_kernel<true><<<dim3((unsigned)dim.cmax, (unsigned)n), kFrontThreads, kFrontLds, st>>>(fb);
       } else {
@@ -1747,6 +1832,12 @@
   const int nh = p.nh, phase = p.phase;
   const bool fused = tail_fusable(n, P, train);
   const bool front = fused && front_fusable(n, P, A);
+  const bool gather = front_gathers(n, P, A, B, train);
+  for (int t = 0; t < n && !gather; ++t)
+    if (wants_gather(A[t])) {
+      tt_set_error("tt_towers_mlp_fwd: gather fields set on a pass that cannot gather (tt_towers_fwd_gathers says which can)");
+      return TT_ERR_UNSUPPORTED;
+    }
   if (phase != 2 && !front) {
     GemmNT nt[TT_MAX_SIDES];
     for (int t = 0; t < n; ++t) {
@@ -1767,7 +1858,7 @@
     const BlockDims dim = block_dims(p, i);
     if (phase != 2 && !(front && tail))
       if (int rc = launch_layer_nt(p, i, tail ? nd : nullptr)) return rc;
-    if (tail) return fwd_narrow_tail(p, i, bs, nd, front, dim);
+    if (tail) return fwd_narrow_tail(p, i, bs, nd, front, gather, dim);
     if (train) {
       if (phase != 2) {
         bn_stats_partial_kernel<<<dim3((unsigned)tt_cdiv(dim.hmax, 64), (unsigned)dim.cmax, (unsigned)n), kThreads, 0, st>>>(bs);
@@ -1794,6 +1885,15 @@
     if (A[t]->emb_packed)
       if (int rc = tt_score_pack_bf16(ctx, A[t]->emb, B, P[t]->d_out, A[t]->emb_pack_scale, A[t]->emb_packed, stream)) return rc;
   return TT_OK;
+}
+
+int tt_towers_fwd_gathers(int32_t n, const tt_tower_params* const* P, const tt_tower_acts* const* A, int64_t B, int32_t train) {
+  if (n < 1 || n > TT_MAX_SIDES || !P || !A) return 0;
+  for (int t = 0; t < n; ++t)
+    if (!P[t] || !A[t] || P[t]->n_hidden < 0 || P[t]->n_hidden > TT_MAX_HIDDEN || !A[t]->dense || !A[t]->x) return 0;
+  for (int t = 0; t < n; ++t)
+    if (P[t]->n_hidden != P[0]->n_hidden || P[t]->compute_dtype != P[0]->compute_dtype) return 0;
+  return front_gathers(n, P, A, B, train) ? 1 : 0;
 }
 
 int tt_towers_mlp_bwd(tt_ctx* ctx, int32_t n, const tt_tower_params* const* P, const tt_tower_acts* const* A,
diff --git a/jodalrob-twotower_amd/ops.py b/jodalrob-twotower_amd/ops.py
--- a/jodalrob-twotower_amd/ops.py
+++ b/jodalrob-twotower_amd/ops.py
@@ -409,6 +409,13 @@
     with _timed("tt_towers_mlp_fwd"):
         L.check(L.load().tt_towers_mlp_fwd(L.ctx(dev), n, P, A, B, int(train), p_drop, seed, L.ptr(seed_dev), wptrs, wsizes,
                                            L.stream(dev)), "tt_towers_mlp_fwd")
+
+
+def towers_fwd_gathers(params_list, acts_list, B, train) -> bool:
+    n = len(params_list)
+    P = (C.POINTER(L.TowerParams) * n)(*[C.pointer(p) for p in params_list])
+    A = (C.POINTER(L.TowerActs) * n)(*[C.pointer(a) for a in acts_list])
+    return bool(L.load().tt_towers_fwd_gathers(n, P, A, B, int(train)))
 
 
 def towers_bwd(params_list, acts_list, d_embs, grads_list, B, train, p_drop, seed, dev, seed_dev=None):
diff --git a/jodalrob-twotower_amd/towers.py b/jodalrob-twotower_amd/towers.py
--- a/jodalrob-twotower_amd/towers.py
+++ b/jodalrob-twotower_amd/towers.py
@@ -31,10 +31,40 @@
     return (n + 63) // 64 * 64
 
 
+def _one_call(sides, key) -> bool:
+    return len(sides) > 1 and len({(s.B, s.tower.n_hidden) + key(s) for s in sides}) == 1
+
+
+def _fwd_key(s):
+    return (s.train, s.p_drop)
+
+
+def _front_gathers(group, live, store, sm, B) -> bool:
+    sides = [g[0] for g in group]
+    if not all(s.tower.front_gather for s in sides) or any(g[2] for g in group) or len(sides) != len(live) or any(a is not b for a, b in zip(sides, live)):
+        return False
+    if _sync_comm(live) is not None or not (len(live) == 1 or _one_call(live, _fwd_key)):
+        return False
+    Ks = [len(s.tower.categorical_embedder.keys) for s in sides]
+    if sm.dtype != torch.int32 or not sm.is_contiguous() or sm.numel() != B * sum(Ks) or sm.device != store.weight.device or not store.weight.is_contiguous():
+        return False
+    base = 0
+    for s, K in zip(sides, Ks):
+        a = s.acts_struct
+        a.gather_table, a.gather_rows, a.gather_K, a.gather_E = store.weight.data_ptr(), sm.data_ptr() + 4 * base, K, store.weight.shape[1]
+        base += B * K
+    if ops.towers_fwd_gathers([s.tower._params() for s in sides], [s.acts_struct for s in sides], B, sides[0].train):
+        return True
+    for s in sides:
+        a = s.acts_struct
+        a.gather_table, a.gather_rows, a.gather_K, a.gather_E = None, None, 0, 0
+    return False
+
+
 def _run_pass(items, one, many, key, sync):
     sides = [it[0] for it in items]
     comm = _sync_comm(sides)
-    if comm is None and not (len(sides) > 1 and len({(s.B, s.tower.n_hidden) + key(s) for s in sides}) == 1):
+    if comm is None and not _one_call(sides, key):
         for s, *args in items:
             one(s.tower._params(), *args, s.B, s.train, s.p_drop, s.seed, s.emb.device, s.tower._seed_dev)
         return None
@@ -88,6 +118,7 @@
         self.x_dtype = torch.bfloat16 if io in ("x", "both") else torch.float32
         self.dx_dtype = torch.bfloat16 if io in ("dx", "both") else torch.float32
         self.unfused_tail, self.unfused_front, self.unfused_back = settings.tower_unfused_tail, settings.tower_unfused_front, settings.tower_unfused_back
+        self.front_gather = settings.front_gather
         self.categorical_keys = list(categorical_keys)
         self.exchange = None
         self.sync_comm = None
@@ -143,7 +174,7 @@
         for lin, bn in zip(lins, bns):
             tensors += [lin.weight, lin.bias, bn.weight, bn.bias, bn.running_mean, bn.running_var]
         w16 = self._w16
-        key = tuple(t.data_ptr() for t in tensors) + tuple(b.num_batches_tracked.data_ptr() for b in bns) + (self.mlp_dtype, self.x_dtype, self.dx_dtype, self.unfused_tail, self.unfused_front, self.unfused_back) + \
+        key = tuple(t.data_ptr() for t in tensors) + tuple(b.num_batches_tracked.data_ptr() for b in bns) + (self.mlp_dtype, self.x_dtype, self.dx_dtype, self.unfused_tail, self.unfused_front, self.unfused_back, self.front_gather) + \
             ((w16[0].data_ptr(),) + tuple(w.data_ptr() for w in w16[1]) if w16 is not None else ())
         if key != self._struct_key:
             for t in tensors:
@@ -159,7 +190,7 @@
                 compute_dtype=ops.TT_BF16 if self.mlp_dtype == "bf16" else ops.TT_F32,
                 x_dtype=ops.TT_BF16 if self.x_dtype == torch.bfloat16 else ops.TT_F32,
                 dx_dtype=ops.TT_BF16 if self.dx_dtype == torch.bfloat16 else ops.TT_F32,
-                flags=(ops.L.TT_TOWER_UNFUSED_TAIL if self.unfused_tail else 0) | (ops.L.TT_TOWER_UNFUSED_FRONT if self.unfused_front else 0) | (ops.L.TT_TOWER_UNFUSED_BACK if self.unfused_back else 0),
+                flags=(ops.L.TT_TOWER_UNFUSED_TAIL if self.unfused_tail else 0) | (ops.L.TT_TOWER_UNFUSED_FRONT if self.unfused_front else 0) | (ops.L.TT_TOWER_UNFUSED_BACK if self.unfused_back else 0) | (0 if self.front_gather else ops.L.TT_TOWER_UNFUSED_GATHER),
                 w_proj_bf16=None if w16 is None else w16[0], w_bf16=() if w16 is None else w16[1])
             self._struct_key = key
         return self._params_struct
@@ -297,6 +328,7 @@
             if K and B:
                 lookups.setdefault(id(emb.store), []).append((s, emb.lookup_side(values, s.x[:, tw.tower_hidden_dims[0]:]), px is not None))
         plans = []
+        live = [s for s in sides if s.B]
         exch = towers[0].exchange
         ctx.exch, ctx.exch_state = exch, None
         if exch is not None:
@@ -319,7 +351,8 @@
                 rows = None
             elif sm is not None and store.weight.shape[1] % 4 == 0 and all(g[1].out.stride(0) % 4 == 0 for g in group):
                 rows = None
-                ops.embed_lookup_rows(store.weight, sm, [g[1] for g in group], B)
+                if not _front_gathers(group, live, store, sm, B):
+                    ops.embed_lookup_rows(store.weight, sm, [g[1] for g in group], B)
             else:
                 rows = ops.embed_lookup(store.weight, [g[1] for g in group], B, want_rows=grad_on and km is None)
             plans.append([store, [g[0] for g in group], None, rows if km is None else km, grad_on, km is not None])
@@ -336,8 +369,7 @@
                         plan = ops.dedup_plan(rows, store.rows)
                     plan.keep = rows
                 pl[:] = [store, psides, plan]
-        live = [s for s in sides if s.B]
-        keep = _run_pass([(s, s.acts_struct) for s in live], ops.tower_fwd, ops.towers_fwd, lambda s: (s.train, s.p_drop),
+        keep = _run_pass([(s, s.acts_struct) for s in live], ops.tower_fwd, ops.towers_fwd, _fwd_key,
                          (1, "bn_sync_local", "bn_sync_all", "bn_sync_stride", 3))
         for s in live if keep else ():
             s.sync_keep = keep
```

Result: faster. 38.96 million, median of 6 (+2.8%).
